# rachtibat/LRP-eXplains-Transformers

Hardware: AMD Instinct MI355X
Metric: explanations/sec (full AttnLRP backward) Llama-3-8B seq=2048 (higher is better)
Workload: dtype bf16

## Files before the change

### include/lrp_hip.h

```cpp
#ifndef LRP_HIP_H
#define LRP_HIP_H
#include <stdint.h>

#ifdef __cplusplus
extern "C" {
#endif

#define LRP_F32 0
#define LRP_BF16 1

#define LRP_OK 0
#define LRP_EINVAL -1
#define LRP_EALIGN -2
#define LRP_ESHAPE -3
#define LRP_ELAUNCH -4

#define LRP_ACT_SILU 0
#define LRP_ACT_GELU_TANH 1
#define LRP_ACT_GELU 2
#define LRP_ACT_TANH 3

int lrp_version(void);
const char* lrp_build_arch(void);
int lrp_last_hip_error(void);
// ... 56 lines not shown
                         float* rel_out, int M, int H, float w_offset, float eps_add,
                         float eps_lin, int dtype, void* stream);

int lrp_sandwich_norm_ok(int H, int dtype);
int lrp_sandwich_norm_fwd(const void* x, const void* res, const void* w_post, const void* w_pre, void* hsum_out, void* y,
                          float* rstd_post, float* rstd_pre, int M, int H, float eps, float w_offset, int dtype, void* stream);
int lrp_sandwich_norm_bwd(const void* Gres, const void* Gx, const void* w_pre, const float* rstd_pre, const void* w_post,
                          const float* rstd_post, void* Gs_out, void* Ga_out, int M, int H, float w_offset, int dtype, void* stream);
int lrp_qk_norm_rope_fwd(const void* qkv, const void* wq, const void* wk, void* qr, void* kr, float* rstd_q, float* rstd_k,
                         const float* cos_t, const float* sin_t, int64_t rows, int seq, int nq, int nk, int d, int64_t ldqkv,
                         int64_t ldq, int64_t ldk, float eps, float w_offset, int dtype, void* stream);
int lrp_qkv_bwd_pack(const void* dq, const void* dk_h, const void* dv_h, const void* wq, const void* wk, const float* rstd_q,
                     const float* rstd_k, const float* cos_t, const float* sin_t, void* A, int64_t rows, int seq, int nq, int nk, int d,
                     int64_t lddq, int64_t lddk, int64_t lddv, int64_t lda, float w_offset, int dtype, void* stream);

int lrp_layernorm_fwd(const void* x, const void* w, const void* b, void* y, float* mean,
                      float* rstd, int M, int H, float eps, int dtype, void* stream);
int lrp_layernorm_bwd(const void* Gy, const void* y, const void* w, const float* rstd,
                      void* Gx, int M, int H, float eps_y, int dtype, void* stream);
int lrp_layernorm_bwd_plain(const void* Gy, const void* x, const void* w, const float* mean, const float* rstd, void* Gx,
                            int M, int H, int dtype, void* stream);


int lrp_gated_act_fwd(const void* g, const void* u, void* m, int M, int I, int64_t ldg,
                      int64_t ldu, int64_t ldm, int act, int dtype, void* stream);
int lrp_gated_act_bwd(const void* Gm, const void* g, const void* u, void* Ag, void* Au,
                      int M, int I, int64_t ldgm, int64_t ldg, int64_t ldu, int64_t ldag,
                      int64_t ldau, float eps_g, float eps_lin, int act, int dtype, void* stream);
#define LRP_GATED_IL 32
int lrp_gated_act_fwd_il(const void* gu, void* m, int M, int I, int64_t ldgu, int64_t ldm, int act, int dtype, void* stream);
int lrp_gated_act_bwd_il(const void* Gm, const void* gu, void* Agu, int M, int I, int64_t ldgm, int64_t ldgu, int64_t ldagu,
                         float eps_g, float eps_lin, int act, int dtype, void* stream);
int lrp_gemm_gated_coef_ok(int M, int I, int H, int64_t ldx, int64_t ldwgu, int64_t lda, int64_t ldwd, int act, int dtype);
int lrp_gemm_gated_fwd_coef(const void* x, const void* Wgu, const float* rs, void* coef, void* m, int M, int I, int K, int64_t ldx, int64_t ldw,
                            int64_t ldcoef, int64_t ldm, float eps_g, float eps_lin, int act, int dtype, void* stream);
int lrp_gemm_gated_bwd_coef(const void* Adn, const void* Wdn, const void* coef, void* Agu, int M, int I, int K, int64_t lda, int64_t ldw,
                            int64_t ldcoef, int64_t ldagu, int dtype, void* stream);

int lrp_gemm_norm_fused_ok(int M, int N, int K, int64_t lda, int64_t ldb, int nn, int dtype);
int lrp_gemm_res_ssq(const void* x, const void* W, const void* res, void* out, float* ssq, int M, int N, int K, int64_t ldx, int64_t ldw,
                     int64_t ldres, int64_t ldout, int64_t ldssq, void* raw, int64_t ldraw, int dtype, void* stream);
int lrp_rms_rstd(const float* ssq, int parts, int64_t ldssq, int M, int H, float eps, float* rstd, void* stream);
int lrp_gemm_nt_rs(const void* x, const void* W, const float* rs, void* out, int M, int N, int K, int64_t ldx, int64_t ldw, int64_t ldout,
                   int dtype, void* stream);
int lrp_gemm_nt_rs_rope_ok(int M, int N, int K, int64_t ldx, int64_t ldw, int64_t ldout, int seq, int rope_cols, int head_dim, int dtype);
int lrp_gemm_nt_rs_rope(const void* x, const void* W, const float* rs, const float* cos, const float* sin, void* out, int M, int N, int K,
                        int64_t ldx, int64_t ldw, int64_t ldout, int seq, int rope_cols, int head_dim, int dtype, void* stream);
int lrp_gemm_nt_rs_bias(const void* x, const void* W, const float* rs, const void* bias, void* out, int M, int N, int K, int64_t ldx, int64_t ldw,
                        int64_t ldout, int dtype, void* stream);
int lrp_gemm_nt_rs_bias_rope_ok(int M, int N, int K, int64_t ldx, int64_t ldw, int64_t ldout, int seq, int rope_cols, int head_dim, int dtype);
int lrp_gemm_nt_rs_bias_rope(const void* x, const void* W, const float* rs, const void* bias, const float* cos, const float* sin, void* out, int M,
                             int N, int K, int64_t ldx, int64_t ldw, int64_t ldout, int seq, int rope_cols, int head_dim, int dtype, void* stream);
int lrp_gemm_nn_rs(const void* s, const void* W, const float* rs, void* out, int M, int N, int K, int64_t lds, int64_t ldw, int64_t ldout,
                   int dtype, void* stream);
int lrp_gemm_nn_rs_res(const void* s, const void* W, const float* rs, const void* res, void* out, int M, int N, int K, int64_t lds, int64_t ldw,
                       int64_t ldres, int64_t ldout, int dtype, void* stream);

int lrp_act_fwd(const void* x, void* y, int64_t n, int act, int dtype, void* stream);
int lrp_act_bwd(const void* Gy, const void* x, void* Gx, int64_t n, float eps_g, int act,
                int dtype, void* stream);
int lrp_act_grad(const void* Gy, const void* x, void* Gx, int64_t n, int act, int dtype, void* stream);

int lrp_add_bcast(const void* x, const void* y, void* out, int M, int H, int period, int dtype, void* stream);

int lrp_rope_fwd(const void* x, void* xr, const float* cos_t, const float* sin_t, int rows,
                 int seq, int n_heads, int d, int64_t ldx, int64_t ldxr, int dtype, void* stream);
int lrp_rope_bwd(const void* Gr, const void* xr, const void* x, void* A, const float* cos_t,
                 const float* sin_t, int rows, int seq, int n_heads, int d, int64_t ldg,
                 int64_t ldxr, int64_t ldx, int64_t lda, float eps_rope, float eps_lin,
                 int dtype, void* stream);

int lrp_transpose_heads(const void* x, void* xt, int B, int S, int H, int d, int64_t ldx,
                        int64_t ldt, int dtype, void* stream);
int lrp_attn_needs_transposed(int dtype, int d);
int lrp_attn_fwd(const void* q, const void* k, const void* v, const void* v_t, void* o, float* lse,
                 int B, int S, int Hq, int Hkv, int d, int64_t ldq, int64_t ldk, int64_t ldv,
                 int64_t ldt, int64_t ldo, float scale, int causal, int window, int q_begin,
                 const int* row_lo, const int* row_hi, int dtype, void* stream);
int lrp_attn_bwd_prep(const void* Go, const void* o, void* Gho, float* D, int B, int S, int Hq,
                      int d, int64_t ldgo, int64_t ldo, int64_t ldgho, float eps_pv,
                      float factor, int dtype, void* stream);
int lrp_attn_bwd_dq(const void* q, const void* k, const void* v, const void* k_t, const void* Gho,
                    const float* lse, const float* D, void* dq, int B, int S, int Hq, int Hkv,
                    int d, int64_t ldq, int64_t ldk, int64_t ldv, int64_t ldt, int64_t ldgho,
                    int64_t lddq, float scale, float eps_mask, float eps_qk, int causal,
                    int window, int q_begin, const int* row_lo, const int* row_hi, int dtype,
                    void* stream);
int lrp_attn_bwd_dq_d_ok(int dtype, int d);
int lrp_attn_bwd_dq_d(const void* q, const void* k, const void* v, const void* Gho, const void* o, const float* lse, float* D, void* dq,
                      int B, int S, int Hq, int Hkv, int d, int64_t ldq, int64_t ldk, int64_t ldv, int64_t ldgho, int64_t ldo, int64_t lddq,
                      float scale, int causal, int window, const int* row_lo, const int* row_hi, const float* cos_t, const float* sin_t,
                      int dtype, void* stream);
int lrp_gqa_reduce_rope(const void* in, void* out, int64_t rows, int seq, int Hkv, int rep, int d, int64_t ld_in, int64_t ld_out,
                        const float* cos_t, const float* sin_t, int dtype, void* stream);
int lrp_attn_bwd_dkv(const void* q, const void* k, const void* v, const void* q_t, const void* Gho,
                     const void* Gho_t, const float* lse, const float* D, void* dk_h, void* dv_h,
                     int B, int S, int Hq, int Hkv, int d, int64_t ldq, int64_t ldk, int64_t ldv,
                     int64_t ldt, int64_t ldgho, int64_t lddk, int64_t lddv, float scale,
                     float eps_mask, float eps_qk, int causal, int window, int q_begin,
                     const int* row_lo, const int* row_hi, int dtype, void* stream);
int lrp_gqa_reduce(const void* in, void* out, int64_t rows, int Hkv, int rep, int d, int64_t ld_in,
                   int64_t ld_out, int dtype, void* stream);

int lrp_softmax_fwd(const void* x, void* p, int64_t rows, int n, float inv_temp, int dtype,
                    void* stream);
int lrp_softmax_rule_bwd(const void* x, const void* p, const void* Rp, void* Rx, int64_t rows,
                         int n, float inv_temp, int dtype, void* stream);
int lrp_add2_rule_bwd(const void* a, const void* b, const void* R, void* Ra, void* Rb,
                      int64_t n, float eps, int dtype, void* stream);

int lrp_readout(const void* emb, const void* G, float* R_tok, int M, int H, int dtype, void* stream);
int64_t lrp_colsum_dot_ws(int B, int S, int N);
int lrp_colsum_dot(const void* x, const void* g, float* out, void* ws, int M, int N, int B, int S, int64_t ldx, int64_t ldg, int dtype,
                   void* stream);
int lrp_head_seed(const void* W_lm, const float* logits, const int* idx, const void* w_norm,
                  const float* rstd_last, void* Gh_last, int B, int V, int H, int64_t ld_logits,
                  float w_offset, float eps_lin, int dtype, void* stream);
int lrp_argmax_rows(const float* logits, int* idx, float* val, int B, int V, int64_t ld, void* stream);
int lrp_transpose(const void* in, void* out, int rows, int cols, int64_t ld_in, int64_t ld_out,
                  int batch, int64_t s_in, int64_t s_out, int dtype, void* stream);
int lrp_cast(const void* in, void* out, int64_t n, int in_dtype, int out_dtype, void* stream);

int64_t lrp_moe_plan_ints(int T, int k, int E);
int lrp_moe_plan(const void* idx, int* plan, int T, int k, int E, void* stream);
int lrp_moe_gate_up_fwd(const void* x, const void* Wgu, const int* plan, void* coef, void* m, int T, int k, int E, int H, int I,
                        int64_t ldx, int64_t ldcoef, int64_t ldm, int act, int dtype, void* stream);
int lrp_moe_down_fwd(const void* m, const void* Wd, const int* plan, void* y, int T, int k, int E, int H, int I, int64_t ldm,
                     int64_t ldy, int dtype, void* stream);
int lrp_moe_combine(const void* rows, const void* w, const int* plan, void* out, int T, int k, int E, int H, int64_t ldr,
                    int64_t ldo, int dtype, void* stream);
int lrp_moe_down_dgrad(const void* G, const void* Wd, const void* coef, const void* m, const void* w, const int* plan, void* Agu,
                       float* gw_part, int T, int k, int E, int H, int I, int64_t ldg, int64_t ldcoef, int64_t ldm,
                       int64_t ldagu, int dtype, void* stream);
int lrp_moe_gw_reduce(const float* gw_part, const int* plan, void* gw, int T, int k, int E, int I, int dtype, void* stream);
int lrp_moe_gate_up_dgrad(const void* Agu, const void* Wgu, const int* plan, void* gx_rows, int T, int k, int E, int H, int I,
                          int64_t ldagu, int64_t ldgx, int dtype, void* stream);

#ifdef __cplusplus
}
#endif
#include "lrp_hip_latent.h"
#include "lrp_hip_moe_router.h"
#include "lrp_hip_mxfp4.h"
#include "lrp_hip_moe_mxfp4.h"
#include "lrp_hip_wgrad.h"
#include "lrp_hip_moe_wgrad.h"
#include "lrp_hip_param_grad.h"
#include "lrp_hip_span.h"
#include "lrp_hip_decode.h"
#include "lrp_hip_decode_site.h"
#include "lrp_hip_mxfp4_stream.h"
#include "lrp_hip_sample.h"
#include "lrp_hip_attn_cp.h"
#endif
```

### lrp-explains-transformers_amd/csrc/attention.hip

```cpp
#include "attention_tiles.hpp"

namespace {

template <typename T, int D, int QSUB>
__global__ __launch_bounds__(ANT, (D >= 256 ? 1 : 2)) void attn_fwd_kernel(
    const T* __restrict__ q, const T* __restrict__ k, const T* __restrict__ vt, T* __restrict__ o, float* __restrict__ lse,
    int S, int Hq, int Hkv, int64_t ldq, int64_t ldk, int64_t ldt, int64_t ldo, float scale, int causal, int window, int q_begin,
    const int* __restrict__ row_lo, const int* __restrict__ row_hi) {
    typedef AT<T> A;
    typedef typename Mma16<T>::frag frag_t;
    constexpr int SZ = A::SZ, CT = A::CT, NC16 = A::NC16, NDC = D * SZ / 64, ND16 = D / 16;
    constexpr int KP = D * SZ;
    constexpr int BQ = 4 * 16 * QSUB;
    extern __shared__ __attribute__((aligned(16))) char smem[];
    char* sK = smem;
    char* sV = smem + CT * KP;

    const int lane = threadIdx.x & 63, wave = threadIdx.x >> 6, g = lane >> 4;
    const int b = blockIdx.z, h = blockIdx.y, hk = h / (Hq / Hkv);
    const int qblk = gridDim.x - 1 - blockIdx.x;
    const int q0 = qblk * BQ, qw = q0 + wave * 16 * QSUB;
    if (q0 + BQ <= q_begin) return;
    const T* qb = q + (int64_t)b * S * ldq + (int64_t)h * D;
    const T* kb = k + (int64_t)b * S * ldk + (int64_t)hk * D;
// ... 872 lines not shown

inline bool al16(const void* p) { return (reinterpret_cast<uintptr_t>(p) & 15) == 0; }

template <auto Kern, typename T, typename... Mid>
void launch_fwd(const AttnCall& c, dim3 grid, int threads, size_t lds, Mid... mid) {
    lrp_launch_lds<Kern>(grid, dim3(threads), lds, lds, c.st, (const T*)c.q, (const T*)c.k, (const T*)c.v_t, (T*)c.o, c.lse_out, c.S, c.Hq, c.Hkv,
                         c.ldq, c.ldk, c.ldt, c.ldo, c.scale, c.causal, c.window, mid..., c.q_begin, c.row_lo, c.row_hi);
}
template <auto Kern, typename T, typename... Mid>
void launch_dq(const AttnCall& c, dim3 grid, int threads, size_t lds, Mid... mid) {
    lrp_launch_lds<Kern>(grid, dim3(threads), lds, lds, c.st, (const T*)c.q, (const T*)c.k, (const T*)c.v, (const T*)c.k_t, (const T*)c.gho, c.lse,
                         c.D, (T*)c.dq, c.S, c.Hq, c.Hkv, c.ldq, c.ldk, c.ldv, c.ldt, c.ldg, c.lddq, c.scale, c.eps_mask, c.eps_qk, c.causal,
                         c.window, mid..., c.q_begin, c.row_lo, c.row_hi);
}
template <auto Kern, typename T, typename... Mid>
void launch_dkv(const AttnCall& c, dim3 grid, int threads, size_t lds, Mid... mid) {
    lrp_launch_lds<Kern>(grid, dim3(threads), lds, lds, c.st, (const T*)c.q, (const T*)c.k, (const T*)c.v, (const T*)c.q_t, (const T*)c.gho,
                         (const T*)c.gho_t, c.lse, c.D, (T*)c.dk, (T*)c.dv, c.S, c.Hq, c.Hkv, c.ldq, c.ldk, c.ldv, c.ldt, c.ldg, c.lddk, c.lddv,
                         c.scale, c.eps_mask, c.eps_qk, c.causal, c.window, mid..., c.q_begin, c.row_lo, c.row_hi);
}

}

static inline bool use_attn32(int dtype, int d) { return dtype == LRP_BF16 && (d == 64 || d == 96 || d == 128 || d == 256); }
extern "C" int lrp_attn_needs_transposed(int dtype, int d) { return use_attn32(dtype, d) ? 0 : 1; }

#define ATT_DISPATCH_D(T, d, ...)                                   \
    if ((size_t)d * sizeof(T) < 64) return LRP_ESHAPE;              \
    if (sizeof(T) == 2 && d != 32) return LRP_ESHAPE;               \
    switch (d) {                                                    \
        case 16: if constexpr (sizeof(T) == 4) { constexpr int DD = 16; __VA_ARGS__ } break;   \
        case 32: { constexpr int DD = 32; __VA_ARGS__ } break;      \
        case 64: if constexpr (sizeof(T) == 4) { constexpr int DD = 64; __VA_ARGS__ } break;   \
        case 128: if constexpr (sizeof(T) == 4) { constexpr int DD = 128; __VA_ARGS__ } break; \
        case 256: if constexpr (sizeof(T) == 4) { constexpr int DD = 256; __VA_ARGS__ } break; \
        default: return LRP_ESHAPE;                                 \
    }

template <typename T> static bool attn_8wave(const AttnCall& c) {
    constexpr int SZ = sizeof(T), CT = 128 / SZ;
    return (c.ldt % CT) == 0 && ((size_t)c.d * SZ >= 64) && c.d <= 128;
}

template <typename T>
static int attn_fwd_t(const AttnCall& c) {
    constexpr int SZ = sizeof(T), CT = 128 / SZ;
    if (attn_8wave<T>(c)) {
        ATT_DISPATCH_D(T, c.d, {
            if constexpr (DD <= 128) {
                const size_t lds = 2 * (2 * (size_t)128 * DD);
                const int rep = c.Hq / c.Hkv;
                if ((int64_t)c.B * c.Hq * ((c.S + 255) / 256) >= 512)
                    launch_fwd<attn_fwd_v2_kernel<T, DD, 2>, T>(c, dim3(xcd_group_grid(c.B * c.Hkv, rep * ((c.S + 255) / 256))), 512, lds, c.B);
                else
                    launch_fwd<attn_fwd_v2_kernel<T, DD, 1>, T>(c, dim3(xcd_group_grid(c.B * c.Hkv, rep * ((c.S + 127) / 128))), 512, lds, c.B);
            }
        })
        return lrp_check_launch();
    }
    ATT_DISPATCH_D(T, c.d, {
        constexpr int QSUB = (DD >= 256) ? 1 : 2;
        constexpr int BQ = 64 * QSUB;
        launch_fwd<attn_fwd_kernel<T, DD, QSUB>, T>(c, dim3((c.S + BQ - 1) / BQ, c.Hq, c.B), ANT, (size_t)CT * DD * SZ + (size_t)DD * 128);
    })
    return lrp_check_launch();
}

static int attn_common_check(int B, int S, int Hq, int Hkv, int d, int dtype, float scale = 1.f) {
    if (!(scale > 0.f)) return LRP_EINVAL;
    if (B < 0 || S < 0 || Hq < 1 || Hkv < 1 || (Hq % Hkv) || d < 16) return LRP_EINVAL;
    if (dtype != LRP_F32 && dtype != LRP_BF16) return LRP_EINVAL;
    if (B > 65535 || Hq > 65535) return LRP_ESHAPE;
    return LRP_OK;
}

extern "C" int lrp_attn_fwd(const void* q, const void* k, const void* v, const void* v_t, void* o, float* lse, int B, int S,
                            int Hq, int Hkv, int d, int64_t ldq, int64_t ldk, int64_t ldv, int64_t ldt, int64_t ldo, float scale,
                            int causal, int window, int q_begin, const int* row_lo, const int* row_hi, int dtype, void* stream) {
    if ((row_lo == nullptr) != (row_hi == nullptr)) return LRP_EINVAL;
    if (!q || !k || !o || !lse) return LRP_EINVAL;
    int rc = attn_common_check(B, S, Hq, Hkv, d, dtype, scale);
    if (rc) return rc;
    if (B == 0 || S == 0) return LRP_OK;
    const int epc = dtype == LRP_F32 ? 4 : 8;
    const bool a32 = use_attn32(dtype, d);
    if (a32) {
        if (!v) return LRP_EINVAL;
        if (!al16(q) || !al16(k) || !al16(v) || !al16(o) || (ldq % epc) || (ldk % epc) || (ldv % epc) || (ldo % 4)) return LRP_EALIGN;
    } else {
        if (!v_t) return LRP_EINVAL;
        if (!al16(q) || !al16(k) || !al16(v_t) || !al16(o) || (ldq % epc) || (ldk % epc) || (ldt % epc) || (ldo % 4) || ldt < S) return LRP_EALIGN;
    }
    AttnCall c = {};
    c.q = q; c.k = k; c.v = v; c.v_t = v_t; c.o = o; c.lse_out = lse;
    c.B = B; c.S = S; c.Hq = Hq; c.Hkv = Hkv; c.d = d;
    c.ldq = ldq; c.ldk = ldk; c.ldv = ldv; c.ldt = ldt; c.ldo = ldo;
    c.scale = scale; c.causal = causal; c.window = window; c.q_begin = q_begin;
    c.row_lo = row_lo; c.row_hi = row_hi; c.st = (hipStream_t)stream;
    if (a32) return lrp_attn32_fwd(c);
    return dtype == LRP_F32 ? attn_fwd_t<float>(c) : attn_fwd_t<bf16_t>(c);
}

template <typename T>
static int attn_dq_t(const AttnCall& c) {
    constexpr int SZ = sizeof(T), CT = 128 / SZ;
    if (attn_8wave<T>(c)) {
        ATT_DISPATCH_D(T, c.d, {
            if constexpr (DD <= 128) {
                const size_t lds = 2 * (3 * (size_t)128 * DD);
                dim3 grid(xcd_group_grid(c.B * c.Hkv, (c.Hq / c.Hkv) * ((c.S + 127) / 128)));
                lrp_with_bool(c.eps_mask != 0.f || c.eps_qk != 0.f, [&](auto ex) {
                    launch_dq<attn_bwd_dq_v2_kernel<T, DD, decltype(ex)::value>, T>(c, grid, 512, lds, c.B);
                });
            }
        })
        return lrp_check_launch();
    }
    ATT_DISPATCH_D(T, c.d, {
        launch_dq<attn_bwd_dq_kernel<T, DD>, T>(c, dim3((c.S + 63) / 64, c.Hq, c.B), ANT, 2 * (size_t)CT * DD * SZ + (size_t)DD * 128);
    })
    return lrp_check_launch();
}

extern "C" int lrp_attn_bwd_dq(const void* q, const void* k, const void* v, const void* k_t, const void* Gho,
                               const float* lse, const float* D, void* dq, int B, int S, int Hq, int Hkv, int d,
                               int64_t ldq, int64_t ldk, int64_t ldv, int64_t ldt, int64_t ldgho, int64_t lddq, float scale,
                               float eps_mask, float eps_qk, int causal, int window, int q_begin, const int* row_lo, const int* row_hi, int dtype, void* stream) {
    if ((row_lo == nullptr) != (row_hi == nullptr)) return LRP_EINVAL;
    if (!q || !k || !v || !Gho || !lse || !D || !dq) return LRP_EINVAL;
    int rc = attn_common_check(B, S, Hq, Hkv, d, dtype, scale);
    if (rc) return rc;
    if (B == 0 || S == 0) return LRP_OK;
    const int epc = dtype == LRP_F32 ? 4 : 8;
    if (!al16(q) || !al16(k) || !al16(v) || !al16(Gho) || !al16(dq) || (ldq % epc) || (ldk % epc) ||
        (ldv % epc) || (ldgho % epc) || (lddq % 4)) return LRP_EALIGN;
    const bool a32 = use_attn32(dtype, d);
    if (!a32) {
        if (!k_t) return LRP_EINVAL;
        if (!al16(k_t) || (ldt % epc) || ldt < S) return LRP_EALIGN;
    }
    AttnCall c = {};
    c.q = q; c.k = k; c.v = v; c.gho = Gho; c.lse = lse; c.D = D;
    c.B = B; c.S = S; c.Hq = Hq; c.Hkv = Hkv; c.d = d;
    c.ldq = ldq; c.ldk = ldk; c.ldv = ldv; c.ldg = ldgho; c.ldt = ldt;
    c.scale = scale; c.eps_mask = eps_mask; c.eps_qk = eps_qk; c.causal = causal; c.window = window; c.q_begin = q_begin;
    c.row_lo = row_lo; c.row_hi = row_hi; c.st = (hipStream_t)stream;
    c.dq = dq; c.lddq = lddq; c.k_t = k_t;
    if (a32) return lrp_attn32_dq(c);
    return dtype == LRP_F32 ? attn_dq_t<float>(c) : attn_dq_t<bf16_t>(c);
}

extern "C" int lrp_attn_bwd_dq_d_ok(int dtype, int d) { return (use_attn32(dtype, d) && d != 256) ? 1 : 0; }

extern "C" int lrp_attn_bwd_dq_d(const void* q, const void* k, const void* v, const void* Gho, const void* o, const float* lse, float* D,
                                 void* dq, int B, int S, int Hq, int Hkv, int d, int64_t ldq, int64_t ldk, int64_t ldv, int64_t ldgho,
                                 int64_t ldo, int64_t lddq, float scale, int causal, int window, const int* row_lo, const int* row_hi,
                                 const float* cos_t, const float* sin_t, int dtype, void* stream) {
    if ((cos_t == nullptr) != (sin_t == nullptr)) return LRP_EINVAL;
    if (cos_t && d != 64 && d != 128) return LRP_ESHAPE;
    if ((row_lo == nullptr) != (row_hi == nullptr)) return LRP_EINVAL;
    if (!q || !k || !v || !Gho || !o || !lse || !D || !dq) return LRP_EINVAL;
    int rc = attn_common_check(B, S, Hq, Hkv, d, dtype, scale);
    if (rc) return rc;
    if (!lrp_attn_bwd_dq_d_ok(dtype, d)) return LRP_ESHAPE;
    if (B == 0 || S == 0) return LRP_OK;
    if (!al16(q) || !al16(k) || !al16(v) || !al16(Gho) || !al16(o) || !al16(dq) || (ldq % 8) || (ldk % 8) || (ldv % 8) || (ldgho % 8) ||
        (ldo % 8) || (lddq % 4)) return LRP_EALIGN;
    AttnCall c = {};
    c.q = q; c.k = k; c.v = v; c.gho = Gho; c.lse = lse; c.D = nullptr;
    c.B = B; c.S = S; c.Hq = Hq; c.Hkv = Hkv; c.d = d;
    c.ldq = ldq; c.ldk = ldk; c.ldv = ldv; c.ldg = ldgho;
    c.scale = scale; c.causal = causal; c.window = window;
    c.row_lo = row_lo; c.row_hi = row_hi; c.st = (hipStream_t)stream;
    c.dq = dq; c.lddq = lddq; c.ofw = o; c.ldo = ldo; c.Dout = D; c.cos_t = cos_t; c.sin_t = sin_t;
    return lrp_attn32_dq(c);
}

template <typename T>
static int attn_dkv_t(const AttnCall& c) {
    constexpr int SZ = sizeof(T), CT = 128 / SZ;
    if (attn_8wave<T>(c) && c.S >= 1) {
        ATT_DISPATCH_D(T, c.d, {
            if constexpr (DD <= 128) {
                const size_t lds = 2 * (4 * (size_t)128 * DD + 512);
                dim3 grid(xcd_group_grid(c.B * c.Hq, (c.S + 127) / 128));
                lrp_with_bool(c.eps_mask != 0.f || c.eps_qk != 0.f, [&](auto ex) {
                    launch_dkv<attn_bwd_dkv_v2_kernel<T, DD, decltype(ex)::value>, T>(c, grid, 512, lds, c.B);
                });
            }
        })
        return lrp_check_launch();
    }
    ATT_DISPATCH_D(T, c.d, {
        launch_dkv<attn_bwd_dkv_kernel<T, DD>, T>(c, dim3((c.S + 63) / 64, c.Hq, c.B), ANT, 2 * (size_t)CT * DD * SZ + 2 * (size_t)DD * 128);
    })
    return lrp_check_launch();
}

extern "C" int lrp_attn_bwd_dkv(const void* q, const void* k, const void* v, const void* q_t, const void* Gho,
                                const void* Gho_t, const float* lse, const float* D, void* dk_h, void* dv_h, int B, int S,
                                int Hq, int Hkv, int d, int64_t ldq, int64_t ldk, int64_t ldv, int64_t ldt, int64_t ldgho,
                                int64_t lddk, int64_t lddv, float scale, float eps_mask, float eps_qk, int causal, int window,
                                int q_begin, const int* row_lo, const int* row_hi, int dtype, void* stream) {
    if ((row_lo == nullptr) != (row_hi == nullptr)) return LRP_EINVAL;
    if (!q || !k || !v || !Gho || !lse || !D || !dk_h || !dv_h) return LRP_EINVAL;
    int rc = attn_common_check(B, S, Hq, Hkv, d, dtype, scale);
    if (rc) return rc;
    if (B == 0 || S == 0) return LRP_OK;
    const int epc = dtype == LRP_F32 ? 4 : 8;
    if (!al16(q) || !al16(k) || !al16(v) || !al16(Gho) || !al16(dk_h) || !al16(dv_h) ||
        (ldq % epc) || (ldk % epc) || (ldv % epc) || (ldgho % epc) || (lddk % 4) || (lddv % 4)) return LRP_EALIGN;
    const bool a32 = use_attn32(dtype, d);
    if (!a32) {
        if (!q_t || !Gho_t) return LRP_EINVAL;
        if (!al16(q_t) || !al16(Gho_t) || (ldt % epc) || ldt < S) return LRP_EALIGN;
    }
    AttnCall c = {};
    c.q = q; c.k = k; c.v = v; c.gho = Gho; c.lse = lse; c.D = D;
    c.B = B; c.S = S; c.Hq = Hq; c.Hkv = Hkv; c.d = d;
    c.ldq = ldq; c.ldk = ldk; c.ldv = ldv; c.ldg = ldgho; c.ldt = ldt;
    c.scale = scale; c.eps_mask = eps_mask; c.eps_qk = eps_qk; c.causal = causal; c.window = window; c.q_begin = q_begin;
    c.row_lo = row_lo; c.row_hi = row_hi; c.st = (hipStream_t)stream;
    c.dk = dk_h; c.dv = dv_h; c.lddk = lddk; c.lddv = lddv; c.q_t = q_t; c.gho_t = Gho_t;
    if (a32) return lrp_attn32_dkv(c);
    return dtype == LRP_F32 ? attn_dkv_t<float>(c) : attn_dkv_t<bf16_t>(c);
}

extern "C" int lrp_transpose_heads(const void* x, void* xt, int B, int S, int H, int d, int64_t ldx, int64_t ldt,
                                   int dtype, void* stream) {
    if (!x || !xt || B < 0 || S < 0 || H < 1 || d < 1 || ldt < S) return LRP_EINVAL;
    if (B == 0 || S == 0) return LRP_OK;
    if ((int64_t)B * H > 65535 || (S + 63) / 64 > 65535) return LRP_ESHAPE;
    hipStream_t st = (hipStream_t)stream;
    dim3 grid((d + 63) / 64, (S + 63) / 64, B * H), block(256);
    const bool vec = dtype == LRP_BF16 && (d % 8) == 0 && (S % 8) == 0 && (ldx % 8) == 0 && (ldt % 8) == 0 && al16(x) && al16(xt);
    if (vec) hipLaunchKernelGGL(transpose_heads_vec_kernel, grid, block, 0, st, (const bf16_t*)x, (bf16_t*)xt, S, H, d, ldx, ldt);
    else if (dtype == LRP_F32) hipLaunchKernelGGL((transpose_heads_kernel<float>), grid, block, 0, st, (const float*)x, (float*)xt, S, H, d, ldx, ldt);
    else if (dtype == LRP_BF16) hipLaunchKernelGGL((transpose_heads_kernel<bf16_t>), grid, block, 0, st, (const bf16_t*)x, (bf16_t*)xt, S, H, d, ldx, ldt);
    else return LRP_EINVAL;
    return lrp_check_launch();
}

extern "C" int lrp_gqa_reduce(const void* in, void* out, int64_t rows, int Hkv, int rep, int d, int64_t ld_in,
                              int64_t ld_out, int dtype, void* stream) {
    if (!in || !out || rows < 0 || Hkv < 1 || rep < 1 || d < 1) return LRP_EINVAL;
    if (rows == 0) return LRP_OK;
    const int epc = dtype == LRP_F32 ? 4 : 8;
    if (dtype != LRP_F32 && dtype != LRP_BF16) return LRP_EINVAL;
    if (!al16(in) || !al16(out) || (d % epc) || (ld_in % epc) || (ld_out % epc)) return LRP_EALIGN;
    hipStream_t st = (hipStream_t)stream;
    const int64_t work = rows * Hkv * (d / epc);
    int64_t nb = (work + 255) / 256;
    if (nb > 2048) nb = 2048;
    if (dtype == LRP_F32) hipLaunchKernelGGL((gqa_reduce_kernel<float>), dim3((unsigned)nb), dim3(256), 0, st, (const float*)in, (float*)out, rows, Hkv, rep, d, ld_in, ld_out);
    else hipLaunchKernelGGL((gqa_reduce_kernel<bf16_t>), dim3((unsigned)nb), dim3(256), 0, st, (const bf16_t*)in, (bf16_t*)out, rows, Hkv, rep, d, ld_in, ld_out);
    return lrp_check_launch();
}

extern "C" int lrp_gqa_reduce_rope(const void* in, void* out, int64_t rows, int seq, int Hkv, int rep, int d, int64_t ld_in, int64_t ld_out,
                                   const float* cos_t, const float* sin_t, int dtype, void* stream) {
    if (!in || !out || !cos_t || !sin_t || rows < 0 || seq < 1 || Hkv < 1 || rep < 1 || d < 2 || (d & 1)) return LRP_EINVAL;
    if (rows == 0) return LRP_OK;
    if (dtype != LRP_F32 && dtype != LRP_BF16) return LRP_EINVAL;
    const int epc = dtype == LRP_F32 ? 4 : 8;
    if (!al16(in) || !al16(out) || ((d / 2) % epc) || (ld_in % epc) || (ld_out % epc)) return LRP_EALIGN;
    hipStream_t st = (hipStream_t)stream;
    const int64_t work = rows * Hkv * (d / 2 / epc);
    int64_t nb = (work + 255) / 256;
    if (nb > 2048) nb = 2048;
    if (dtype == LRP_F32) hipLaunchKernelGGL((gqa_reduce_rope_kernel<float>), dim3((unsigned)nb), dim3(256), 0, st, (const float*)in, (float*)out, rows, seq, Hkv, rep, d, ld_in, ld_out, cos_t, sin_t);
    else hipLaunchKernelGGL((gqa_reduce_rope_kernel<bf16_t>), dim3((unsigned)nb), dim3(256), 0, st, (const bf16_t*)in, (bf16_t*)out, rows, seq, Hkv, rep, d, ld_in, ld_out, cos_t, sin_t);
    return lrp_check_launch();
}
```

### lrp-explains-transformers_amd/csrc/attention32.hip

```cpp
#include "attention32_tiles.hpp"

namespace attn32 {

template <int DH>
__global__ __launch_bounds__(NWQ * 64, 2) void fwd_kernel(
    const bf16_t* __restrict__ q, const bf16_t* __restrict__ k, const bf16_t* __restrict__ v, bf16_t* __restrict__ o,
    float* __restrict__ lse, int S, int Hq, int Hkv, int64_t ldq, int64_t ldk, int64_t ldv, int64_t ldo, float scale,
    int causal, int window, int B, int q_begin, const int* __restrict__ row_lo, const int* __restrict__ row_hi) {
    constexpr int BQ = NWQ * 32, STAGE = 2 * TILE, NK = DH / 16, ND32 = DH / 32;
    extern __shared__ __attribute__((aligned(16))) char smem[];
    const int lane = threadIdx.x & 63, l31 = lane & 31, hi = lane >> 5;
    const int wave = __builtin_amdgcn_readfirstlane(threadIdx.x >> 6);
    const int rep = Hq / Hkv, nqb = (S + BQ - 1) / BQ;
    int bhk, item;
    if (!xcd_group_decode(blockIdx.x, B * Hkv, rep * nqb, bhk, item)) return;
    const int b = bhk / Hkv, hk = bhk % Hkv, h = hk * rep + item % rep;
    const int qblk = nqb - 1 - item / rep;
    const int q0 = qblk * BQ, qw = q0 + wave * 32, qi = qw + l31;
    if (q0 + BQ <= q_begin) return;
    const bf16_t* kb_ = k + (int64_t)b * S * ldk + (int64_t)hk * DH;
    const bf16_t* vb_ = v + (int64_t)b * S * ldv + (int64_t)hk * DH;

    bf16x8 qf[NK];
    load_row_frags<DH>(qf, q + (int64_t)b * S * ldq + (int64_t)h * DH, ldq, qi, S, hi);
    int ivlo = 0, ivhi = S;
    if (row_lo != nullptr && qi < S) { ivlo = row_lo[(int64_t)b * S + qi]; ivhi = row_hi[(int64_t)b * S + qi]; }
    f32x16 oacc[ND32];
#pragma unroll
    for (int db = 0; db < ND32; ++db) oacc[db] = zero16();
    float m_run = -INFINITY, l_run = 0.f;
    const float c1 = scale * LRP_LOG2E;
    int kend = S;
    if (causal) kend = min(S, q0 + BQ);
    int kbeg = 0;
    if (window > 0) { kbeg = q0 - window + 1; kbeg = kbeg < 0 ? 0 : (kbeg / CT) * CT; }
    IvWave ivw = {0, S, 0, S};
    if (row_lo != nullptr) {
        int* ivsh = reinterpret_cast<int*>(smem);
        ivw = iv_wave(ivlo, ivhi, qi < S, wave, ivsh);
        __syncthreads();
        int glo, ghi;
        iv_fold<NWQ>(ivsh, glo, ghi);
        __syncthreads();
        kbeg = max(kbeg, (min(glo, S) / CT) * CT);
        kend = min(kend, ghi);
    }

    auto stage = [&](int kt0, int buf) {
        char* sb = smem + buf * STAGE;
        stage_tile<NWQ, DH>(kb_, ldk, kt0, S, sb, wave, lane);
        stage_tile<NWQ, DH>(vb_, ldv, kt0, S, sb + TILE, wave, lane);
    };
    if (kbeg < kend) stage(kbeg, 0);
    __syncthreads();
    uint32_t arm[NK], atr[NDX][2];
    {
        const uint32_t sbase = lds_addr(smem);
        LaneAddr la;
        la.init(lane);
#pragma unroll
        for (int ks = 0; ks < NK; ++ks) arm[ks] = sbase + la.rm[ks];
#pragma unroll
        for (int db = 0; db < ND32; ++db) { atr[db][0] = sbase + la.tr[db][0]; atr[db][1] = sbase + la.tr[db][1]; }
    }
    int cur = 0;
    for (int kt0 = kbeg; kt0 < kend; kt0 += CT) {
        if (kt0 + CT < kend) stage(kt0 + CT, cur ^ 1);
        const bool dead = (causal && kt0 > qw + 31) || kt0 >= ivw.hi_max || kt0 + CT <= ivw.lo_min;
        if (!dead) {
            f32x16 st[2] = {zero16(), zero16()};
            bf16x8 f0[3], f1[3];
            A32_RD128(f0[0], arm[0], 0); A32_RD128(f1[0], arm[0], 32 * KP);
            A32_RD128(f0[1], arm[1], 0); A32_RD128(f1[1], arm[1], 32 * KP);
            sfor<0, NK>([&](auto ksc) {
                constexpr int ks = decltype(ksc)::value, cu = ks % 3, nx = (ks + 2) % 3;
                if constexpr (ks + 2 < NK) {
                    A32_RD128(f0[nx], arm[ks + 2], 0); A32_RD128(f1[nx], arm[ks + 2], 32 * KP);
                    A32_WAIT(4, "+v"(f0[cu]), "+v"(f1[cu]));
                } else if constexpr (ks + 1 < NK) {
                    A32_WAIT(2, "+v"(f0[cu]), "+v"(f1[cu]));
                } else {
                    A32_WAIT(0, "+v"(f0[cu]), "+v"(f1[cu]));
                }
                st[0] = mfma32(f0[cu], qf[ks], st[0]);
                st[1] = mfma32(f1[cu], qf[ks], st[1]);
                A32_FENCE();
            });
            u32x2 tv0[2][NDX][2], tv1[2][NDX][2];
            tr_group<ND32, TILE>(tv0[0], atr);
            tr_group<ND32, TILE + 16 * KP>(tv0[1], atr);
            A32_FENCE();
            const bool need_mask = (kt0 + CT > S) || (causal && kt0 + CT - 1 > qw) || (window > 0) ||
                                   (row_lo != nullptr && !(kt0 >= ivw.lo_max && kt0 + CT <= ivw.hi_min));
            if (need_mask) {
#pragma unroll
                for (int kb = 0; kb < 2; ++kb)
#pragma unroll
                    for (int r = 0; r < 16; ++r)
                        st[kb][r] = visible(qi, kt0 + kb * 32 + crow(r, hi), S, causal, window, ivlo, ivhi) ? st[kb][r] : -INFINITY;
            }
            float mx = -INFINITY;
#pragma unroll
            for (int kb = 0; kb < 2; ++kb)
#pragma unroll
                for (int r = 0; r < 16; ++r) mx = fmaxf(mx, st[kb][r]);
            mx = half_max(mx);
            float m_new = m_run;
            if (__any((mx - m_run) * c1 > 8.f || (m_run == -INFINITY && mx != -INFINITY))) m_new = fmaxf(m_run, mx);
            const float m_use = (m_new == -INFINITY) ? 0.f : m_new;
            const float nm2 = -m_use * c1;
            float rs = 0.f;
#pragma unroll
            for (int kb = 0; kb < 2; ++kb)
#pragma unroll
                for (int r = 0; r < 16; ++r) {
                    const float p = fast_exp2(__builtin_fmaf(st[kb][r], c1, nm2));
                    st[kb][r] = p;
                    rs += p;
                }
            rs = half_sum(rs);
            if (__any(m_new != m_run)) {
                const float alpha = fast_exp2((m_run - m_use) * c1);
                l_run = l_run * alpha + rs;
#pragma unroll
                for (int db = 0; db < ND32; ++db) oacc[db] *= alpha;
            } else l_run += rs;
            m_run = m_new;
            const bf16x8 p00 = pack8(st[0], 0), p01 = pack8(st[0], 1), p10 = pack8(st[1], 0), p11 = pack8(st[1], 1);
            A32_FENCE();
            tr_group<ND32, TILE + 32 * KP>(tv1[0], atr);
            wait_tr2<ND32, 2 * ND32>(tv0[0], tv0[1]);
#pragma unroll
            for (int db = 0; db < ND32; ++db) oacc[db] = mfma32(join_tr(tv0[0][db][0], tv0[0][db][1]), p00, oacc[db]);
            A32_FENCE();
            tr_group<ND32, TILE + 48 * KP>(tv1[1], atr);
#pragma unroll
            for (int db = 0; db < ND32; ++db) oacc[db] = mfma32(join_tr(tv0[1][db][0], tv0[1][db][1]), p01, oacc[db]);
            A32_FENCE();
            wait_tr<ND32, 2 * ND32>(tv1[0]);
#pragma unroll
            for (int db = 0; db < ND32; ++db) oacc[db] = mfma32(join_tr(tv1[0][db][0], tv1[0][db][1]), p10, oacc[db]);
            A32_FENCE();
            wait_tr<ND32, 0>(tv1[1]);
#pragma unroll
            for (int db = 0; db < ND32; ++db) oacc[db] = mfma32(join_tr(tv1[1][db][0], tv1[1][db][1]), p11, oacc[db]);
            A32_FENCE();
        }
        asm volatile("s_waitcnt vmcnt(0)" ::: "memory");
        __syncthreads();
        {
            const uint32_t delta = cur ? (uint32_t)-STAGE : (uint32_t)STAGE;
#pragma unroll
            for (int ks = 0; ks < NK; ++ks) arm[ks] += delta;
#pragma unroll
            for (int db = 0; db < ND32; ++db) { atr[db][0] += delta; atr[db][1] += delta; }
        }
        cur ^= 1;
    }
    const float inv = (l_run > 0.f) ? 1.f / l_run : 0.f;
    store_rows<DH>(o + (int64_t)b * S * ldo + (int64_t)h * DH, ldo, qi, S, oacc, inv, hi);
    if (hi == 0 && qi < S) lse[((int64_t)b * Hq + h) * S + qi] = m_run * scale + __logf(l_run);
}

template <bool EXPL, int DH>
__global__ __launch_bounds__(NWQ * 64, 2) void dq_kernel(
    const bf16_t* __restrict__ q, const bf16_t* __restrict__ k, const bf16_t* __restrict__ v, const bf16_t* __restrict__ gho,
    const float* __restrict__ lse, const float* __restrict__ Dd, bf16_t* __restrict__ dq, int S, int Hq, int Hkv, int64_t ldq,
    int64_t ldk, int64_t ldv, int64_t ldg, int64_t lddq, float scale, float eps_mask, float eps_qk, int causal, int window,
    int B, int q_begin, const int* __restrict__ row_lo, const int* __restrict__ row_hi, const bf16_t* __restrict__ ofw, int64_t ldo,
    float* __restrict__ Dout, const float* __restrict__ rope_cos, const float* __restrict__ rope_sin) {
    constexpr int BQ = NWQ * 32, STAGE = 2 * TILE, NK = DH / 16, ND32 = DH / 32;
    extern __shared__ __attribute__((aligned(16))) char smem[];
    const int lane = threadIdx.x & 63, l31 = lane & 31, hi = lane >> 5;
    const int wave = __builtin_amdgcn_readfirstlane(threadIdx.x >> 6);
    const int rep = Hq / Hkv, nqb = (S + BQ - 1) / BQ;
    int bhk, item;
    if (!xcd_group_decode(blockIdx.x, B * Hkv, rep * nqb, bhk, item)) return;
    const int b = bhk / Hkv, hk = bhk % Hkv, h = hk * rep + item % rep;
    const int qblk = nqb - 1 - item / rep;
    const int q0 = qblk * BQ, qw = q0 + wave * 32, qi = qw + l31;
    if (q0 + BQ <= q_begin) return;
    const bf16_t* kb_ = k + (int64_t)b * S * ldk + (int64_t)hk * DH;
    const bf16_t* vb_ = v + (int64_t)b * S * ldv + (int64_t)hk * DH;

    bf16x8 qf[NK], gf[NK];
    load_row_frags<DH>(qf, q + (int64_t)b * S * ldq + (int64_t)h * DH, ldq, qi, S, hi);
    load_row_frags<DH>(gf, gho + (int64_t)b * S * ldg + (int64_t)h * DH, ldg, qi, S, hi);
    const float lse2 = ((qi < S) ? lse[((int64_t)b * Hq + h) * S + qi] : 0.f) * LRP_LOG2E;
    float Dq;
    if (ofw != nullptr) {
        bf16x8 of[NK];
        load_row_frags<DH>(of, ofw + (int64_t)b * S * ldo + (int64_t)h * DH, ldo, qi, S, hi);
        float sd = 0.f;
#pragma unroll
        for (int ks = 0; ks < NK; ++ks)
#pragma unroll
            for (int e = 0; e < 8; ++e) sd += (float)gf[ks][e] * (float)of[ks][e];
        sd += __shfl_xor(sd, 32);
        Dq = sd;
        if (hi == 0 && qi < S) Dout[((int64_t)b * Hq + h) * S + qi] = sd;
    } else Dq = (qi < S) ? Dd[((int64_t)b * Hq + h) * S + qi] : 0.f;
    int ivlo = 0, ivhi = S;
    if (row_lo != nullptr && qi < S) { ivlo = row_lo[(int64_t)b * S + qi]; ivhi = row_hi[(int64_t)b * S + qi]; }
    f32x16 acc[ND32];
#pragma unroll
    for (int db = 0; db < ND32; ++db) acc[db] = zero16();
    const float c1 = scale * LRP_LOG2E;
    int kend = S;
    if (causal) kend = min(S, q0 + BQ);
    int kbeg = 0;
    if (window > 0) { kbeg = q0 - window + 1; kbeg = kbeg < 0 ? 0 : (kbeg / CT) * CT; }
    IvWave ivw = {0, S, 0, S};
    if (row_lo != nullptr) {
        int* ivsh = reinterpret_cast<int*>(smem);
        ivw = iv_wave(ivlo, ivhi, qi < S, wave, ivsh);
        __syncthreads();
        int glo, ghi;
        iv_fold<NWQ>(ivsh, glo, ghi);
        __syncthreads();
        kbeg = max(kbeg, (min(glo, S) / CT) * CT);
        kend = min(kend, ghi);
    }

    auto stage = [&](int kt0, int buf) {
        char* sb = smem + buf * STAGE;
        stage_tile<NWQ, DH>(kb_, ldk, kt0, S, sb, wave, lane);
        stage_tile<NWQ, DH>(vb_, ldv, kt0, S, sb + TILE, wave, lane);
    };
    if (kbeg < kend) stage(kbeg, 0);
    __syncthreads();
    uint32_t arm[NK], atr[NDX][2];
    {
        const uint32_t sbase = lds_addr(smem);
        LaneAddr la;
        la.init(lane);
#pragma unroll
        for (int ks = 0; ks < NK; ++ks) arm[ks] = sbase + la.rm[ks];
#pragma unroll
        for (int db = 0; db < ND32; ++db) { atr[db][0] = sbase + la.tr[db][0]; atr[db][1] = sbase + la.tr[db][1]; }
    }
#ifdef A32_TIMELINE
    uint32_t tl_acc[8] = {0, 0, 0, 0, 0, 0, 0, 0}, tl_prev = (uint32_t)__builtin_readcyclecounter();
    const uint32_t tl_start = tl_prev;
#endif
    int cur = 0;
    for (int kt0 = kbeg; kt0 < kend; kt0 += CT) {
        if (kt0 + CT < kend) stage(kt0 + CT, cur ^ 1);
        A32_TS(0);
        sfor<0, 2>([&](auto kbc) {
            constexpr int kb = decltype(kbc)::value, KO = kb * 32 * KP;
            const int kk0 = kt0 + kb * 32;
            if ((causal && kk0 > qw + 31) || kk0 >= S || kk0 >= ivw.hi_max || kk0 + 32 <= ivw.lo_min) return;
            f32x16 st = zero16(), dp = zero16();
            bf16x8 fk[3], fv[3];
            A32_RD128(fk[0], arm[0], KO); A32_RD128(fv[0], arm[0], KO + TILE);
            A32_RD128(fk[1], arm[1], KO); A32_RD128(fv[1], arm[1], KO + TILE);
            sfor<0, NK>([&](auto ksc) {
                constexpr int ks = decltype(ksc)::value, cu = ks % 3, nx = (ks + 2) % 3;
                if constexpr (ks + 2 < NK) {
                    A32_RD128(fk[nx], arm[ks + 2], KO); A32_RD128(fv[nx], arm[ks + 2], KO + TILE);
                    A32_WAIT(4, "+v"(fk[cu]), "+v"(fv[cu]));
                } else if constexpr (ks + 1 < NK) {
                    A32_WAIT(2, "+v"(fk[cu]), "+v"(fv[cu]));
                } else {
                    A32_WAIT(0, "+v"(fk[cu]), "+v"(fv[cu]));
                }
                st = mfma32(fk[cu], qf[ks], st);
                dp = mfma32(fv[cu], gf[ks], dp);
                A32_FENCE();
            });
            A32_TS(1);
            u32x2 tk[2][NDX][2];
            tr_group<ND32, KO>(tk[0], atr);
            tr_group<ND32, KO + 16 * KP>(tk[1], atr);
            A32_FENCE();
            const bool masked = (kk0 + 32 > S) || (causal && kk0 + 31 > qw) || (window > 0) ||
                                (row_lo != nullptr && !(kk0 >= ivw.lo_max && kk0 + 32 <= ivw.hi_min));
            if (masked) {
#pragma unroll
                for (int r = 0; r < 16; ++r) {
                    const float s_raw = st[r];
                    float p = fast_exp2(__builtin_fmaf(s_raw, c1, -lse2));
                    if (!visible(qi, kk0 + crow(r, hi), S, causal, window, ivlo, ivhi)) p = 0.f;
                    st[r] = lrp_ds<EXPL>(s_raw, p, dp[r], Dq, scale, eps_mask, eps_qk);
                }
            } else {
#pragma unroll
                for (int r = 0; r < 16; ++r) {
                    const float s_raw = st[r];
                    const float p = fast_exp2(__builtin_fmaf(s_raw, c1, -lse2));
                    st[r] = lrp_ds<EXPL>(s_raw, p, dp[r], Dq, scale, eps_mask, eps_qk);
                }
            }
            const bf16x8 df0 = pack8(st, 0), df1 = pack8(st, 1);
            A32_FENCE();
            A32_TS(2);
            wait_tr<ND32, 2 * ND32>(tk[0]);
#pragma unroll
            for (int db = 0; db < ND32; ++db) acc[db] = mfma32(join_tr(tk[0][db][0], tk[0][db][1]), df0, acc[db]);
            A32_FENCE();
            wait_tr<ND32, 0>(tk[1]);
#pragma unroll
            for (int db = 0; db < ND32; ++db) acc[db] = mfma32(join_tr(tk[1][db][0], tk[1][db][1]), df1, acc[db]);
            A32_FENCE();
            A32_TS(3);
        });
        asm volatile("s_waitcnt vmcnt(0)" ::: "memory");
        A32_TS(4);
        __syncthreads();
        A32_TS(5);
        {
            const uint32_t delta = cur ? (uint32_t)-STAGE : (uint32_t)STAGE;
#pragma unroll
            for (int ks = 0; ks < NK; ++ks) arm[ks] += delta;
#pragma unroll
            for (int db = 0; db < ND32; ++db) { atr[db][0] += delta; atr[db][1] += delta; }
        }
        cur ^= 1;
    }
    const float omul = EXPL ? 1.f : 0.5f * scale;
    if constexpr (!EXPL && (DH == 64 || DH == 128)) {
        if (rope_cos != nullptr) {
            const int pos = qi < S ? qi : 0;
            const float* pc = rope_cos + (int64_t)pos * DH;
            const float* ps = rope_sin + (int64_t)pos * DH;
#pragma unroll
            for (int db = 0; db < ND32 / 2; ++db)
#pragma unroll
                for (int i = 0; i < 4; ++i) {
                    const int c = db * 32 + 8 * i + 4 * hi;
                    const f32x4 c1 = *reinterpret_cast<const f32x4*>(pc + c), s1 = *reinterpret_cast<const f32x4*>(ps + c);
#pragma unroll
                    for (int e = 0; e < 4; ++e) {
                        const float g1 = acc[db][4 * i + e], g2 = acc[db + ND32 / 2][4 * i + e];
                        acc[db][4 * i + e] = g1 * c1[e] + g2 * s1[e];
                        acc[db + ND32 / 2][4 * i + e] = g2 * c1[e] - g1 * s1[e];
                    }
                }
        }
    }
    store_rows<DH>(dq + (int64_t)b * S * lddq + (int64_t)h * DH, lddq, qi, S, acc, omul, hi);
#ifdef A32_TIMELINE
    if (lane == 0 && qw < S) {
        uint32_t* w = reinterpret_cast<uint32_t*>(dq + ((int64_t)b * S + qw) * lddq + (int64_t)h * DH);
#pragma unroll
        for (int i = 0; i < 6; ++i) w[i] = tl_acc[i];
        w[6] = (uint32_t)__builtin_readcyclecounter() - tl_start;
        w[7] = (uint32_t)((kend - kbeg + CT - 1) / CT);
    }
#endif
}

template <bool EXPL, int DH, bool IV>
__global__ __launch_bounds__(512, 2) void dkv_kernel(
    const bf16_t* __restrict__ q, const bf16_t* __restrict__ k, const bf16_t* __restrict__ v, const bf16_t* __restrict__ gho,
    const float* __restrict__ lse, const float* __restrict__ Dd, bf16_t* __restrict__ dk, bf16_t* __restrict__ dv, int S, int Hq,
    int Hkv, int64_t ldq, int64_t ldk, int64_t ldv, int64_t ldg, int64_t lddk, int64_t lddv, float scale, float eps_mask,
    float eps_qk, int causal, int window, int B, int q_begin, const int* __restrict__ row_lo, const int* __restrict__ row_hi) {
    constexpr int BK = NW * 32, STAGE = 2 * TILE + 512, VROWS = 32 * KP, NK = DH / 16, ND32 = DH / 32;
    extern __shared__ __attribute__((aligned(16))) char smem[];
    const int lane = threadIdx.x & 63, l31 = lane & 31, hi = lane >> 5;
    const int wave = __builtin_amdgcn_readfirstlane(threadIdx.x >> 6);
    int bh, kblk;
    if (!xcd_item_major_decode(blockIdx.x, B * Hq, (S + BK - 1) / BK, bh, kblk)) return;
    const int b = bh / Hq, h = bh % Hq, hk = h / (Hq / Hkv);
    const int k0 = kblk * BK, kw = k0 + wave * 32, ki = kw + l31;
    const bf16_t* qb_ = q + (int64_t)b * S * ldq + (int64_t)h * DH;
    const bf16_t* gb_ = gho + (int64_t)b * S * ldg + (int64_t)h * DH;
    const float* lse_b = lse + ((int64_t)b * Hq + h) * S;
    const float* D_b = Dd + ((int64_t)b * Hq + h) * S;
    const int* rlo_b = (IV && row_lo) ? row_lo + (int64_t)b * S : nullptr;
    const int* rhi_b = (IV && row_lo) ? row_hi + (int64_t)b * S : nullptr;
    int* const ivtab = reinterpret_cast<int*>(smem + 2 * STAGE + NW * VROWS);

    bf16x8 kf[NK];
    load_row_frags<DH>(kf, k + (int64_t)b * S * ldk + (int64_t)hk * DH, ldk, ki, S, hi);
    char* sVw = smem + 2 * STAGE + wave * VROWS;
    {
        const bf16_t* vbase = v + (int64_t)b * S * ldv + (int64_t)hk * DH;
        const __amdgpu_buffer_rsrc_t rs = __builtin_amdgcn_make_buffer_rsrc((void*)vbase, 0, (int)(((int64_t)(S - 1) * ldv + DH) * 2), 0x00020000);
        const int rl = lane >> 4, slot = lane & 15;
#pragma unroll
        for (int g = 0; g < 8; ++g) {
            const int chunk_ = slot ^ ((rl << 2) | (g & 3));
            const int voff = (DH == 128 || chunk_ < DH / 8) ? (int)(rl * ldv * 2) + (chunk_ << 4) : A32_OOB;
            __builtin_amdgcn_raw_ptr_buffer_load_lds(rs, (lds_ptr_t)(sVw + g * 1024), 16, voff, (int)((int64_t)(kw + g * 4) * ldv * 2), 0, 0);
        }
    }
    f32x16 dkacc[ND32], dvacc[ND32];
#pragma unroll
    for (int db = 0; db < ND32; ++db) { dkacc[db] = zero16(); dvacc[db] = zero16(); }
    const float c1 = scale * LRP_LOG2E;
    int qbeg = 0, qend = S;
    if (causal) qbeg = (k0 / CT) * CT;
    if (window > 0) qend = min(S, k0 + BK - 1 + window);
    if (q_begin > qbeg) qbeg = (q_begin / CT) * CT;
    if (rlo_b != nullptr) {
        int qlo, qhi;
        iv_block_table<NW>(rlo_b, rhi_b, S, k0, BK, wave, lane, ivtab, reinterpret_cast<int*>(smem), qlo, qhi);
        qbeg = max(qbeg, (min(qlo, S) / CT) * CT);
        qend = min(qend, qhi);
    }

    auto stage = [&](int qt0, int buf) {
        char* sb = smem + buf * STAGE;
        stage_tile<NW, DH>(qb_, ldq, qt0, S, sb, wave, lane);
        stage_tile<NW, DH>(gb_, ldg, qt0, S, sb + TILE, wave, lane);
        if (wave == 0) stage_stats(lse_b, qt0, S, sb + 2 * TILE, lane);
        if (wave == 1) stage_stats(D_b, qt0, S, sb + 2 * TILE + 256, lane);
    };
    if (qbeg < qend) stage(qbeg, 0);
    __syncthreads();
    uint32_t arm0, avw0, atr[ND32][2], ast;
    {
        const uint32_t sbase = lds_addr(smem);
        LaneAddr la;
        la.init(lane);
        arm0 = sbase + la.rm[0];
        avw0 = arm0 + 2 * STAGE + wave * VROWS;
#pragma unroll
        for (int db = 0; db < ND32; ++db) { atr[db][0] = sbase + la.tr[db][0]; atr[db][1] = sbase + la.tr[db][1]; }
        ast = sbase + 2 * TILE + hi * 16;
    }
#ifdef A32_TIMELINE
    uint32_t tl_acc[8] = {0, 0, 0, 0, 0, 0, 0, 0}, tl_prev = (uint32_t)__builtin_readcyclecounter();
    const uint32_t tl_start = tl_prev;
#endif
    int cur = 0;
    for (int qt0 = qbeg; qt0 < qend; qt0 += CT) {
        if (qt0 + CT < qend) stage(qt0 + CT, cur ^ 1);
        A32_TS(0);
        sfor<0, 2>([&](auto qbc) {
            constexpr int qb = decltype(qbc)::value, QO = qb * 32 * KP, SO = qb * 128;
            const int qq0 = qt0 + qb * 32;
            bool live = !((causal && qq0 + 31 < kw) || qq0 >= S);
            bool iv_mask = false;
            if (live && rlo_b != nullptr) {
                int t0_, t1_, t2_, t3_;
                iv_row(ivtab, qq0 >> 5, t0_, t1_, t2_, t3_);
                if (t1_ <= kw || t0_ >= kw + 32) live = false;
                iv_mask = !(t2_ <= kw && t3_ >= kw + 32);
            }
            if (!live) return;
            f32x16 st = zero16(), dp = zero16();
            f32x4 sl[2], sd[2];
            constexpr int PD = 2, RS = PD + 1;
            bf16x8 fq[RS], fg[RS], fv[RS];
            static_assert(PD < NK, "read-ahead deeper than the contraction");
            static_assert(PD == 2, "the prologue below issues the reads of steps 0 .. PD - 1");
#define A32_P1_PRO(pk)                                                                                          \
    {                                                                                                           \
        const uint32_t aq = frag_addr<(pk)>(arm0), av = frag_addr<(pk)>(avw0);                                  \
        A32_RD128(fq[pk], aq, QO); A32_RD128(fg[pk], aq, QO + TILE); A32_RD128(fv[pk], av, 0);                  \
    }
            A32_P1_PRO(0) A32_P1_PRO(1)
#undef A32_P1_PRO
            sfor<0, NK>([&](auto ksc) {
                constexpr int ks = decltype(ksc)::value, cu = ks % RS, nx = (ks + PD) % RS;
                constexpr int ahead = (ks + PD < NK ? PD : NK - 1 - ks);
                if constexpr (ks + PD < NK) {
                    const uint32_t aq = frag_addr<ks + PD>(arm0), av = frag_addr<ks + PD>(avw0);
                    A32_RD128(fq[nx], aq, QO); A32_RD128(fg[nx], aq, QO + TILE); A32_RD128(fv[nx], av, 0);
                }
                if constexpr (ks == NK - 2) { A32_RD128(sl[0], ast, SO); A32_RD128(sd[0], ast, SO + 256); }
                constexpr int nw = 3 * ahead + (ks >= NK - 2 ? 2 : 0);
                static_assert(nw <= 14, "lgkmcnt is a 4-bit counter");
                asm volatile("s_waitcnt lgkmcnt(%[n])" : "+v"(fq[cu]), "+v"(fg[cu]), "+v"(fv[cu]) : [n] "n"(nw));
                st = mfma32(fq[cu], kf[ks], st);
                dp = mfma32(fg[cu], fv[cu], dp);
                A32_FENCE();
            });
            A32_TS(1);
            u32x2 tg[2][2], tq[2][2];
#define A32_TRG(slot, jj, dbb)                                                                                        \
    A32_RDTR(tg[slot][0], atr[dbb][0], QO + TILE + (jj) * 16 * KP); A32_RDTR(tg[slot][1], atr[dbb][1], QO + TILE + (jj) * 16 * KP); \
    A32_RDTR(tq[slot][0], atr[dbb][0], QO + (jj) * 16 * KP); A32_RDTR(tq[slot][1], atr[dbb][1], QO + (jj) * 16 * KP)
#define A32_TIE(sl_) "+v"(tg[sl_][0]), "+v"(tg[sl_][1]), "+v"(tq[sl_][0]), "+v"(tq[sl_][1])
#define A32_DKV_STEP(g, wait_stmt)                                                                     \
    {                                                                                                  \
        constexpr int j_ = (g) / ND32, db_ = (g) % ND32, sl_ = (g)&1;                                  \
        wait_stmt;                                                                                     \
        dvacc[db_] = mfma32(join_tr(tg[sl_][0], tg[sl_][1]), pf[j_], dvacc[db_]);                      \
        dkacc[db_] = mfma32(join_tr(tq[sl_][0], tq[sl_][1]), df[j_], dkacc[db_]);                      \
        A32_FENCE();                                                                                   \
    }
            const bool masked = (qq0 + 32 > S) || (causal && qq0 < kw + 31) || (window > 0) || iv_mask;
            bf16x8 pf[2], df[2];
            auto elementwise = [&](auto ic) {
                constexpr int i = decltype(ic)::value, cu = i & 1, nx = cu ^ 1;
                if constexpr (i == 0) {
                    A32_RD128(sl[nx], ast, SO + 32); A32_RD128(sd[nx], ast, SO + 32 + 256);
                    A32_WAIT(6, "+v"(sl[cu]), "+v"(sd[cu]));
                } else if constexpr (i == 1) {
                    A32_RD128(sl[nx], ast, SO + 64); A32_RD128(sd[nx], ast, SO + 64 + 256);
                    A32_WAIT(2, "+v"(sl[cu]), "+v"(sd[cu]), A32_TIE(0));
                } else if constexpr (i == 2) {
                    A32_RD128(sl[nx], ast, SO + 96); A32_RD128(sd[nx], ast, SO + 96 + 256);
                    A32_WAIT(6, "+v"(sl[cu]), "+v"(sd[cu]));
                } else if constexpr (ND32 == 3) {
                    A32_WAIT(0, "+v"(sl[cu]), "+v"(sd[cu]), A32_TIE(1));
                } else {
                    A32_WAIT(0, "+v"(sl[cu]), "+v"(sd[cu]), A32_TIE(0));
                }
                float pe[4];
#pragma unroll
                for (int e = 0; e < 4; ++e) pe[e] = fast_exp2(__builtin_fmaf(st[4 * i + e], c1, -(sl[cu][e] * LRP_LOG2E)));
                if (masked) {
#pragma unroll
                    for (int e = 0; e < 4; ++e) {
                        const int qi = qq0 + 8 * i + 4 * hi + e;
                        int ivlo = 0, ivhi = S;
                        if constexpr (IV) { if (rlo_b != nullptr && qi < S) { ivlo = rlo_b[qi]; ivhi = rhi_b[qi]; } }
                        pe[e] = ((qi < S) & visible(qi, ki, S, causal, window, ivlo, ivhi)) ? pe[e] : 0.f;
                    }
                }
#pragma unroll
                for (int e = 0; e < 4; ++e) {
                    const int r = 4 * i + e;
                    pf[i >> 1][4 * (i & 1) + e] = (bf16_t)pe[e];
                    df[i >> 1][4 * (i & 1) + e] = (bf16_t)lrp_ds<EXPL>(st[r], pe[e], dp[r], sd[cu][e], scale, eps_mask, eps_qk);
                }
                A32_FENCE();
            };
            A32_TRG(0, 0, 0);
            A32_FENCE();
            elementwise(IC<0>{});
            elementwise(IC<1>{});
            if constexpr (ND32 == 4) {
                A32_TS(2);
                A32_TRG(1, 0, 1);
                A32_DKV_STEP(0, (void)0);
                A32_TRG(0, 0, 2);
                A32_DKV_STEP(1, A32_WAIT(4, A32_TIE(1)));
                A32_TRG(1, 0, 3);
                A32_DKV_STEP(2, A32_WAIT(4, A32_TIE(0)));
                A32_TRG(0, 1, 0);
                A32_DKV_STEP(3, A32_WAIT(4, A32_TIE(1)));
                A32_TS(3);
                elementwise(IC<2>{});
                elementwise(IC<3>{});
                A32_TS(2);
                A32_TRG(1, 1, 1);
                A32_DKV_STEP(4, (void)0);
                A32_TRG(0, 1, 2);
                A32_DKV_STEP(5, A32_WAIT(4, A32_TIE(1)));
                A32_TRG(1, 1, 3);
                A32_DKV_STEP(6, A32_WAIT(4, A32_TIE(0)));
                A32_DKV_STEP(7, A32_WAIT(0, A32_TIE(1)));
                A32_TS(3);
            } else if constexpr (ND32 == 3) {
                A32_TRG(1, 0, 1);
                A32_DKV_STEP(0, (void)0);
                A32_TRG(0, 0, 2);
                A32_DKV_STEP(1, A32_WAIT(4, A32_TIE(1)));
                A32_TRG(1, 1, 0);
                A32_DKV_STEP(2, A32_WAIT(4, A32_TIE(0)));
                elementwise(IC<2>{});
                elementwise(IC<3>{});
                A32_TRG(0, 1, 1);
                A32_DKV_STEP(3, (void)0);
                A32_TRG(1, 1, 2);
                A32_DKV_STEP(4, A32_WAIT(4, A32_TIE(0)));
                A32_DKV_STEP(5, A32_WAIT(0, A32_TIE(1)));
            } else {
                A32_TRG(1, 0, 1);
                A32_DKV_STEP(0, (void)0);
                A32_TRG(0, 1, 0);
                A32_DKV_STEP(1, A32_WAIT(4, A32_TIE(1)));
                elementwise(IC<2>{});
                elementwise(IC<3>{});
                A32_TRG(1, 1, 1);
                A32_DKV_STEP(2, (void)0);
                A32_DKV_STEP(3, A32_WAIT(0, A32_TIE(1)));
            }
#undef A32_DKV_STEP
#undef A32_TIE
#undef A32_TRG
        });
        asm volatile("s_waitcnt vmcnt(0)" ::: "memory");
        A32_TS(4);
        __syncthreads();
        A32_TS(5);
        {
            const uint32_t delta = cur ? (uint32_t)-STAGE : (uint32_t)STAGE;
            arm0 += delta;
#pragma unroll
            for (int db = 0; db < ND32; ++db) { atr[db][0] += delta; atr[db][1] += delta; }
            ast += delta;
        }
        cur ^= 1;
    }
    store_rows<DH>(dk + (int64_t)b * S * lddk + (int64_t)h * DH, lddk, ki, S, dkacc, EXPL ? 1.f : 0.5f * scale, hi);
    store_rows<DH>(dv + (int64_t)b * S * lddv + (int64_t)h * DH, lddv, ki, S, dvacc, 1.f, hi);
#ifdef A32_TIMELINE
    asm volatile("s_waitcnt vmcnt(0)" ::: "memory");
    if (lane == 0 && kw < S) {
        uint32_t* w = reinterpret_cast<uint32_t*>(dk + ((int64_t)b * S + kw) * lddk + (int64_t)h * DH);
#pragma unroll
        for (int i = 0; i < 6; ++i) w[i] = tl_acc[i];
        w[6] = (uint32_t)__builtin_readcyclecounter() - tl_start;
        w[7] = (uint32_t)((qend - qbeg + CT - 1) / CT);
    }
#endif
}


namespace d256 {

constexpr int D2 = 256, KP2 = 512, CT2 = 32, TILE2 = CT2 * KP2, NK2 = 16, ND2 = 8, NW2 = 4;

LRP_DEVICE void stage_tile2(const bf16_t* base, int64_t ld, int row0, int S, char* lds, int wave, int lane) {
    const __amdgpu_buffer_rsrc_t rs = __builtin_amdgcn_make_buffer_rsrc((void*)base, 0, (int)(((int64_t)(S - 1) * ld + D2) * 2), 0x00020000);
    const int rl = lane >> 5, slot = lane & 31;
#pragma unroll
    for (int g = 0; g < 4; ++g) {
        const int grp = g * NW2 + wave;
        const int rot = ((2 * (wave & 1) + rl) << 2) | ((2 * g + (wave >> 1)) & 3);
        const int voff = (int)(rl * ld * 2) + ((slot ^ rot) << 4);
        __builtin_amdgcn_raw_ptr_buffer_load_lds(rs, (lds_ptr_t)(lds + grp * 1024), 16, voff, (int)((int64_t)(row0 + 2 * grp) * ld * 2), 0, 0);
    }
}
LRP_DEVICE void stage_block2(const bf16_t* base, int64_t ld, int row0, int S, char* lds, int lane) {
    const __amdgpu_buffer_rsrc_t rs = __builtin_amdgcn_make_buffer_rsrc((void*)base, 0, (int)(((int64_t)(S - 1) * ld + D2) * 2), 0x00020000);
    const int rl = lane >> 5, slot = lane & 31;
#pragma unroll
    for (int g = 0; g < 16; ++g) {
        const int rot = ((2 * (g & 1) + rl) << 2) | ((g >> 1) & 3);
        const int voff = (int)(rl * ld * 2) + ((slot ^ rot) << 4);
        __builtin_amdgcn_raw_ptr_buffer_load_lds(rs, (lds_ptr_t)(lds + g * 1024), 16, voff, (int)((int64_t)(row0 + 2 * g) * ld * 2), 0, 0);
    }
}
LRP_DEVICE uint32_t rm_base(int lane) {
    const int l31 = lane & 31, hi = lane >> 5;
    return (uint32_t)(l31 * KP2 + ((hi ^ rot4(l31)) << 4));
}
LRP_DEVICE uint32_t tr_base(int lane, int half) {
    const int l31 = lane & 31, hi = lane >> 5, i16 = lane & 15;
    const int r = half * 8 + 4 * hi + (i16 >> 2);
    const int chunk = ((l31 >> 4) << 1) + ((i16 & 3) >> 1);
    return (uint32_t)(r * KP2 + ((chunk ^ rot4(r)) << 4) + 8 * (i16 & 1));
}
template <int X> LRP_DEVICE uint32_t xor_addr(uint32_t a0) {
    if constexpr (X == 0) return a0;
    else {
        uint32_t r;
        asm volatile("v_xor_b32 %0, %1, %2" : "=v"(r) : "n"(X), "v"(a0));
        return r;
    }
}
LRP_DEVICE void load_row_frags2(bf16x8* f, const bf16_t* base, int64_t ld, int row, int S, int hi) {
    const bool ok = row < S;
#pragma unroll
    for (int ks = 0; ks < NK2; ++ks) {
        if (ok) f[ks] = *reinterpret_cast<const bf16x8*>(base + (int64_t)row * ld + ks * 16 + hi * 8);
        else {
            u32x4 z = {0, 0, 0, 0};
            f[ks] = __builtin_bit_cast(bf16x8, z);
        }
    }
}
LRP_DEVICE void store_rows2(bf16_t* base, int64_t ld, int row, int S, const f32x16* acc, float mul, int hi) {
    attn32::store_rows<D2>(base, ld, row, S, acc, mul, hi);
}
#define A2_UNIT(dst, a0, a1, J, DBH, OFF)                                                                            \
    {                                                                                                                \
        const uint32_t b0_ = xor_addr<((DBH) * 4 + 0) << 6>(a0), c0_ = xor_addr<((DBH) * 4 + 0) << 6>(a1);           \
        const uint32_t b1_ = xor_addr<((DBH) * 4 + 1) << 6>(a0), c1_ = xor_addr<((DBH) * 4 + 1) << 6>(a1);           \
        const uint32_t b2_ = xor_addr<((DBH) * 4 + 2) << 6>(a0), c2_ = xor_addr<((DBH) * 4 + 2) << 6>(a1);           \
        const uint32_t b3_ = xor_addr<((DBH) * 4 + 3) << 6>(a0), c3_ = xor_addr<((DBH) * 4 + 3) << 6>(a1);           \
        A32_RDTR(dst[0][0], b0_, (OFF) + (J) * 16 * KP2); A32_RDTR(dst[0][1], c0_, (OFF) + (J) * 16 * KP2);          \
        A32_RDTR(dst[1][0], b1_, (OFF) + (J) * 16 * KP2); A32_RDTR(dst[1][1], c1_, (OFF) + (J) * 16 * KP2);          \
        A32_RDTR(dst[2][0], b2_, (OFF) + (J) * 16 * KP2); A32_RDTR(dst[2][1], c2_, (OFF) + (J) * 16 * KP2);          \
        A32_RDTR(dst[3][0], b3_, (OFF) + (J) * 16 * KP2); A32_RDTR(dst[3][1], c3_, (OFF) + (J) * 16 * KP2);          \
    }
#define A2_UNITV(t) "+v"(t[0][0]), "+v"(t[0][1]), "+v"(t[1][0]), "+v"(t[1][1]), "+v"(t[2][0]), "+v"(t[2][1]), "+v"(t[3][0]), "+v"(t[3][1])

__global__ __launch_bounds__(NW2 * 64, 1) void fwd256_kernel(
    const bf16_t* __restrict__ q, const bf16_t* __restrict__ k, const bf16_t* __restrict__ v, bf16_t* __restrict__ o,
    float* __restrict__ lse, int S, int Hq, int Hkv, int64_t ldq, int64_t ldk, int64_t ldv, int64_t ldo, float scale,
    int causal, int window, int B, int q_begin, const int* __restrict__ row_lo, const int* __restrict__ row_hi) {
    constexpr int BQ = NW2 * 32, STAGE = 2 * TILE2;
    extern __shared__ __attribute__((aligned(16))) char smem[];
    const int lane = threadIdx.x & 63, l31 = lane & 31, hi = lane >> 5;
    const int wave = __builtin_amdgcn_readfirstlane(threadIdx.x >> 6);
    const int rep = Hq / Hkv, nqb = (S + BQ - 1) / BQ;
    int bhk, item;
    if (!xcd_group_decode(blockIdx.x, B * Hkv, rep * nqb, bhk, item)) return;
    const int b = bhk / Hkv, hk = bhk % Hkv, h = hk * rep + item % rep;
    const int qblk = nqb - 1 - item / rep;
    const int q0 = qblk * BQ, qw = q0 + wave * 32, qi = qw + l31;
    if (q0 + BQ <= q_begin) return;
    const bf16_t* kb_ = k + (int64_t)b * S * ldk + (int64_t)hk * D2;
    const bf16_t* vb_ = v + (int64_t)b * S * ldv + (int64_t)hk * D2;

    bf16x8 qf[NK2];
    load_row_frags2(qf, q + (int64_t)b * S * ldq + (int64_t)h * D2, ldq, qi, S, hi);
    int ivlo = 0, ivhi = S;
    if (row_lo != nullptr && qi < S) { ivlo = row_lo[(int64_t)b * S + qi]; ivhi = row_hi[(int64_t)b * S + qi]; }
    f32x16 oacc[ND2];
#pragma unroll
    for (int db = 0; db < ND2; ++db) oacc[db] = zero16();
    float m_run = -INFINITY, l_run = 0.f;
    const float c1 = scale * LRP_LOG2E;
    int kend = S;
    if (causal) kend = min(S, q0 + BQ);
    int kbeg = 0;
    if (window > 0) { kbeg = q0 - window + 1; kbeg = kbeg < 0 ? 0 : (kbeg / CT2) * CT2; }
    IvWave ivw = {0, S, 0, S};
    if (row_lo != nullptr) {
        int* ivsh = reinterpret_cast<int*>(smem);
        ivw = iv_wave(ivlo, ivhi, qi < S, wave, ivsh);
        __syncthreads();
        int glo, ghi;
        iv_fold<NW2>(ivsh, glo, ghi);
        __syncthreads();
        kbeg = max(kbeg, (min(glo, S) / CT2) * CT2);
        kend = min(kend, ghi);
    }

    auto stage = [&](int kt0, int buf) {
        char* sb = smem + buf * STAGE;
        stage_tile2(kb_, ldk, kt0, S, sb, wave, lane);
        stage_tile2(vb_, ldv, kt0, S, sb + TILE2, wave, lane);
    };
    if (kbeg < kend) stage(kbeg, 0);
    asm volatile("s_waitcnt vmcnt(0)" ::: "memory");
    __syncthreads();
    uint32_t arm = lds_addr(smem) + rm_base(lane), at0 = lds_addr(smem) + tr_base(lane, 0), at1 = lds_addr(smem) + tr_base(lane, 1);
    int cur = 0;
    for (int kt0 = kbeg; kt0 < kend; kt0 += CT2) {
        if (kt0 + CT2 < kend) stage(kt0 + CT2, cur ^ 1);
        const bool dead = (causal && kt0 > qw + 31) || (window > 0 && kt0 + CT2 - 1 <= qw - window) || kt0 >= ivw.hi_max || kt0 + CT2 <= ivw.lo_min;
        if (!dead) {
            f32x16 st = zero16();
            bf16x8 fk[3];
            A32_RD128(fk[0], arm, 0);
            { const uint32_t a_ = xor_addr<1 << 5>(arm); A32_RD128(fk[1], a_, 0); }
            sfor<0, NK2>([&](auto ksc) {
                constexpr int ks = decltype(ksc)::value, cu = ks % 3, nx = (ks + 2) % 3;
                (void)&fk; (void)&arm;
                if constexpr (ks + 2 < NK2) {
                    { const uint32_t a_ = xor_addr<(ks + 2) << 5>(arm); A32_RD128(fk[nx], a_, 0); }
                    A32_WAIT(2, "+v"(fk[cu]));
                } else if constexpr (ks + 1 < NK2) {
// ... 277 lines not shown
                iv_mask = !(t2_ <= kw && t3_ >= kw + 32);
            }
            if (!dead) {
                f32x16 st = zero16(), dp = zero16();
                bf16x8 fq[3];
                A32_RD128(fq[0], arm, 0);
                { const uint32_t a_ = xor_addr<1 << 5>(arm); A32_RD128(fq[1], a_, 0); }
                sfor<0, NK2>([&](auto ksc) {
                    constexpr int ks = decltype(ksc)::value, cu = ks % 3, nx = (ks + 2) % 3;
                    (void)&fq; (void)&arm;
                    if constexpr (ks + 2 < NK2) {
                        { const uint32_t a_ = xor_addr<(ks + 2) << 5>(arm); A32_RD128(fq[nx], a_, 0); }
                        A32_WAIT(2, "+v"(fq[cu]));
                    } else if constexpr (ks + 1 < NK2) {
                        A32_WAIT(1, "+v"(fq[cu]));
                    } else {
                        A32_WAIT(0, "+v"(fq[cu]));
                    }
                    st = mfma32(fq[cu], kf[ks], st);
                    A32_FENCE();
                });
                if constexpr (PASS == 1) {
                    bf16x8 fg[3], fv[3];
                    A32_RD128(fg[0], arm, TILE2); A32_RD128(fv[0], avw, 0);
                    { const uint32_t a_ = xor_addr<1 << 5>(arm), b_ = xor_addr<1 << 5>(avw); A32_RD128(fg[1], a_, TILE2); A32_RD128(fv[1], b_, 0); }
                    sfor<0, NK2>([&](auto ksc) {
                        constexpr int ks = decltype(ksc)::value, cu = ks % 3, nx = (ks + 2) % 3;
                        (void)&fg; (void)&fv; (void)&arm; (void)&avw;
                        if constexpr (ks + 2 < NK2) {
                            { const uint32_t a_ = xor_addr<(ks + 2) << 5>(arm), b_ = xor_addr<(ks + 2) << 5>(avw); A32_RD128(fg[nx], a_, TILE2); A32_RD128(fv[nx], b_, 0); }
                            A32_WAIT(4, "+v"(fg[cu]), "+v"(fv[cu]));
                        } else if constexpr (ks + 1 < NK2) {
                            A32_WAIT(2, "+v"(fg[cu]), "+v"(fv[cu]));
                        } else {
                            A32_WAIT(0, "+v"(fg[cu]), "+v"(fv[cu]));
                        }
                        dp = mfma32(fg[cu], fv[cu], dp);
                        A32_FENCE();
                    });
                }
                constexpr int TOFF = (PASS == 0) ? TILE2 : 0;
                u32x2 tt[2][4][2];
                A2_UNIT(tt[0], at0, at1, 0, 0, TOFF);
                A32_FENCE();
                const bool masked = (qt0 + 32 > S) || (causal && qt0 < kw + 31) || (window > 0 && qt0 + 31 - window >= kw) || iv_mask;
                bf16x8 xf[2];
                f32x4 sl[2], sd[2];
                sfor<0, 2>([&](auto jc) {
                    constexpr int j = decltype(jc)::value;
                    (void)&sl; (void)&sd; (void)&ast;
                    A32_RD128(sl[0], ast, 64 * j); A32_RD128(sl[1], ast, 64 * j + 32);
                    if constexpr (PASS == 1) {
                        A32_RD128(sd[0], ast, 64 * j + 256); A32_RD128(sd[1], ast, 64 * j + 32 + 256);
                        A32_WAIT(0, "+v"(sl[0]), "+v"(sl[1]), "+v"(sd[0]), "+v"(sd[1]));
                    } else {
                        A32_WAIT(0, "+v"(sl[0]), "+v"(sl[1]));
                    }
#pragma unroll
                    for (int ii = 0; ii < 2; ++ii)
#pragma unroll
                        for (int e = 0; e < 4; ++e) {
                            const int i = 2 * j + ii, r = 4 * i + e;
                            const float s_raw = st[r];
                            float p = fast_exp2(__builtin_fmaf(s_raw, c1, -(sl[ii][e] * LRP_LOG2E)));
                            if (masked) {
                                const int qi = qt0 + 8 * i + 4 * hi + e;
                                int ivlo = 0, ivhi = S;
                                if (rlo_b != nullptr && qi < S) { ivlo = rlo_b[qi]; ivhi = rhi_b[qi]; }
                                p = ((qi < S) & visible(qi, ki, S, causal, window, ivlo, ivhi)) ? p : 0.f;
                            }
                            if constexpr (PASS == 0) xf[j][4 * ii + e] = (bf16_t)p;
                            else xf[j][4 * ii + e] = (bf16_t)lrp_ds<EXPL>(s_raw, p, dp[r], sd[ii][e], scale, eps_mask, eps_qk);
                        }
                    A32_FENCE();
                });
                A2_UNIT(tt[1], at0, at1, 0, 1, TOFF);
                A32_WAIT(8, A2_UNITV(tt[0]));
#pragma unroll
                for (int d4 = 0; d4 < 4; ++d4) acc[d4] = mfma32(join_tr(tt[0][d4][0], tt[0][d4][1]), xf[0], acc[d4]);
                A32_FENCE();
                A2_UNIT(tt[0], at0, at1, 1, 0, TOFF);
                A32_WAIT(8, A2_UNITV(tt[1]));
#pragma unroll
                for (int d4 = 0; d4 < 4; ++d4) acc[4 + d4] = mfma32(join_tr(tt[1][d4][0], tt[1][d4][1]), xf[0], acc[4 + d4]);
                A32_FENCE();
                A2_UNIT(tt[1], at0, at1, 1, 1, TOFF);
                A32_WAIT(8, A2_UNITV(tt[0]));
#pragma unroll
                for (int d4 = 0; d4 < 4; ++d4) acc[d4] = mfma32(join_tr(tt[0][d4][0], tt[0][d4][1]), xf[1], acc[d4]);
                A32_FENCE();
                A32_WAIT(0, A2_UNITV(tt[1]));
#pragma unroll
                for (int d4 = 0; d4 < 4; ++d4) acc[4 + d4] = mfma32(join_tr(tt[1][d4][0], tt[1][d4][1]), xf[1], acc[4 + d4]);
                A32_FENCE();
            }
            asm volatile("s_waitcnt vmcnt(0)" ::: "memory");
            __syncthreads();
            {
                const uint32_t delta = cur ? (uint32_t)-STAGE : (uint32_t)STAGE;
                arm += delta; at0 += delta; at1 += delta; ast += delta;
            }
            cur ^= 1;
        }
        if constexpr (PASS == 0) store_rows2(dv + (int64_t)b * S * lddv + (int64_t)h * D2, lddv, ki, S, acc, 1.f, hi);
        else store_rows2(dk + (int64_t)b * S * lddk + (int64_t)h * D2, lddk, ki, S, acc, EXPL ? 1.f : 0.5f * scale, hi);
    });
}

}

constexpr size_t A32_LDS_MAX = 160 * 1024;

template <auto Kern>
static void launch_fwd(const AttnCall& c, int nw, size_t lds) {
    dim3 grid(xcd_group_grid(c.B * c.Hkv, (c.Hq / c.Hkv) * ((c.S + nw * 32 - 1) / (nw * 32))));
    lrp_launch_lds<Kern>(grid, dim3(nw * 64), lds, lds, c.st, (const bf16_t*)c.q, (const bf16_t*)c.k, (const bf16_t*)c.v, (bf16_t*)c.o, c.lse_out,
                         c.S, c.Hq, c.Hkv, c.ldq, c.ldk, c.ldv, c.ldo, c.scale, c.causal, c.window, c.B, c.q_begin, c.row_lo, c.row_hi);
}
template <auto Kern, typename... Tail>
static void launch_dq(const AttnCall& c, int nw, size_t lds, Tail... tail) {
    dim3 grid(xcd_group_grid(c.B * c.Hkv, (c.Hq / c.Hkv) * ((c.S + nw * 32 - 1) / (nw * 32))));
    lrp_launch_lds<Kern>(grid, dim3(nw * 64), lds, lds, c.st, (const bf16_t*)c.q, (const bf16_t*)c.k, (const bf16_t*)c.v, (const bf16_t*)c.gho,
                         c.lse, c.D, (bf16_t*)c.dq, c.S, c.Hq, c.Hkv, c.ldq, c.ldk, c.ldv, c.ldg, c.lddq, c.scale, c.eps_mask, c.eps_qk,
                         c.causal, c.window, c.B, c.q_begin, c.row_lo, c.row_hi, tail...);
}
template <auto Kern>
static void launch_dkv(const AttnCall& c, int nw, size_t lds) {
    dim3 grid(xcd_group_grid(c.B * c.Hq, (c.S + nw * 32 - 1) / (nw * 32)));
    lrp_launch_lds<Kern>(grid, dim3(nw * 64), lds, A32_LDS_MAX, c.st, (const bf16_t*)c.q, (const bf16_t*)c.k, (const bf16_t*)c.v,
                         (const bf16_t*)c.gho, c.lse, c.D, (bf16_t*)c.dk, (bf16_t*)c.dv, c.S, c.Hq, c.Hkv, c.ldq, c.ldk, c.ldv, c.ldg, c.lddk,
                         c.lddv, c.scale, c.eps_mask, c.eps_qk, c.causal, c.window, c.B, c.q_begin, c.row_lo, c.row_hi);
}

}

#define A32_FOR_DH(d, ...)                                     \
    switch (d) {                                               \
        case 64: { constexpr int DH = 64; __VA_ARGS__ } break; \
        case 96: { constexpr int DH = 96; __VA_ARGS__ } break; \
        case 128: { constexpr int DH = 128; __VA_ARGS__ } break; \
        default: return LRP_ESHAPE;                            \
    }

int lrp_attn32_fwd(const AttnCall& c) {
    using namespace attn32;
    if (c.d == 256) launch_fwd<d256::fwd256_kernel>(c, d256::NW2, 2 * (2 * (size_t)d256::TILE2));
    else A32_FOR_DH(c.d, { launch_fwd<fwd_kernel<DH>>(c, NWQ, 2 * (2 * (size_t)TILE)); })
    return lrp_check_launch();
}

int lrp_attn32_dq(const AttnCall& c) {
    using namespace attn32;
    const bool expl = c.eps_mask != 0.f || c.eps_qk != 0.f;
    if (c.d == 256)
        lrp_with_bool(expl, [&](auto ex) { launch_dq<d256::dq256_kernel<decltype(ex)::value>>(c, d256::NW2, 2 * (2 * (size_t)d256::TILE2)); });
    else A32_FOR_DH(c.d, {
        lrp_with_bool(expl, [&](auto ex) {
            launch_dq<dq_kernel<decltype(ex)::value, DH>>(c, NWQ, 2 * (2 * (size_t)TILE), (const bf16_t*)c.ofw, c.ldo, c.Dout, c.cos_t, c.sin_t);
        });
    })
    return lrp_check_launch();
}

int lrp_attn32_dkv(const AttnCall& c) {
    using namespace attn32;
    const bool wide = c.d == 256, expl = c.eps_mask != 0.f || c.eps_qk != 0.f, iv = c.row_lo != nullptr;
    const size_t lds = (wide ? 2 * (2 * (size_t)d256::TILE2 + 512) + (size_t)d256::NW2 * 32 * d256::KP2 : 2 * (2 * (size_t)TILE + 512) + (size_t)NW * 32 * KP) +
                       (iv ? (size_t)((c.S + 31) / 32) * 16 : 0);
    if (lds > A32_LDS_MAX) return LRP_ESHAPE;
    if (wide) lrp_with_bool(expl, [&](auto ex) { launch_dkv<d256::dkv256_kernel<decltype(ex)::value>>(c, d256::NW2, lds); });
    else A32_FOR_DH(c.d, {
        lrp_with_bool(expl, [&](auto ex) {
            lrp_with_bool(iv, [&](auto ivf) { launch_dkv<dkv_kernel<decltype(ex)::value, DH, decltype(ivf)::value>>(c, NW, lds); });
        });
    })
    return lrp_check_launch();
}
```

### lrp-explains-transformers_amd/csrc/attention32_tiles.hpp

```cpp
#pragma once
#include "common.hpp"

namespace attn32 {

typedef __attribute__((ext_vector_type(4))) short s16x4;
typedef __attribute__((address_space(3))) s16x4* lds_s16x4_t;
typedef __attribute__((address_space(3))) void* lds_ptr_t;
typedef const __attribute__((address_space(1))) void* glb_ptr_t;

constexpr int NW = 8;
constexpr int NWQ = 4;
constexpr int CT = 64;
constexpr int KP = 256;
constexpr int TILE = CT * KP;
constexpr int NKX = 8, NDX = 4;
#define LRP_LOG2E 1.4426950408889634f

LRP_DEVICE int rot4(int r) { return ((r & 3) << 2) | ((r >> 2) & 3); }
LRP_DEVICE float fast_exp2(float x) { return __builtin_amdgcn_exp2f(x); }

LRP_DEVICE bool xcd_group_decode(int L, int ngroups, int per_group, int& group, int& item) {
    const int xcd = L & 7, i = L >> 3;
    item = i % per_group;
    group = xcd + 8 * (i / per_group);
    return group < ngroups;
}
LRP_DEVICE bool xcd_item_major_decode(int L, int ngroups, int per_group, int& group, int& item) {
    const int xcd = L & 7, i = L >> 3, gpx = (ngroups + 7) >> 3;
    item = i / gpx;
    group = xcd + 8 * (i % gpx);
    return group < ngroups;
}

constexpr int A32_OOB = 0x40000000;
template <int NWV = NW, int DH = 128>
LRP_DEVICE void stage_tile(const bf16_t* base, int64_t ld, int row0, int S, char* lds, int wave, int lane) {
    const __amdgpu_buffer_rsrc_t rs = __builtin_amdgcn_make_buffer_rsrc((void*)base, 0, (int)(((int64_t)(S - 1) * ld + DH) * 2), 0x00020000);
    const int rl = lane >> 4, slot = lane & 15;
    const int chunk_ = slot ^ ((rl << 2) | (wave & 3));
    const int voff = (DH == 128 || chunk_ < DH / 8) ? (int)(rl * ld * 2) + (chunk_ << 4) : A32_OOB;
#pragma unroll
    for (int g = 0; g < 16 / NWV; ++g) {
        const int grp = g * NWV + wave;
        __builtin_amdgcn_raw_ptr_buffer_load_lds(rs, (lds_ptr_t)(lds + grp * 1024), 16, voff, (int)((int64_t)(row0 + grp * 4) * ld * 2), 0, 0);
    }
}
LRP_DEVICE void stage_stats(const float* base, int r0, int S, char* lds, int lane) {
    int r = r0 + lane;
    r = r < S ? r : S - 1;
    __builtin_amdgcn_global_load_lds((glb_ptr_t)(base + r), (lds_ptr_t)lds, 4, 0, 0);
}

struct LaneAddr {
    uint32_t rm[NKX];
    uint32_t tr[NDX][2];
    LRP_DEVICE void init(int lane) {
        const int l31 = lane & 31, hi = lane >> 5, i16 = lane & 15;
#pragma unroll
        for (int ks = 0; ks < NKX; ++ks) rm[ks] = l31 * KP + (((ks * 2 + hi) ^ rot4(l31)) << 4);
#pragma unroll
        for (int db = 0; db < NDX; ++db)
#pragma unroll
            for (int half = 0; half < 2; ++half) {
                const int r = half * 8 + 4 * hi + (i16 >> 2);
                const int chunk = db * 4 + ((l31 >> 4) << 1) + ((i16 & 3) >> 1);
                tr[db][half] = r * KP + ((chunk ^ rot4(r)) << 4) + 8 * (i16 & 1);
            }
    }
};

LRP_DEVICE bf16x8 lds_frag(const char* tile, uint32_t off) { return *reinterpret_cast<const bf16x8*>(tile + off); }
LRP_DEVICE bf16x8 lds_frag_tr(const char* tile, uint32_t off0, uint32_t off1) {
    const s16x4 a = __builtin_amdgcn_ds_read_tr16_b64_v4i16((lds_s16x4_t)(tile + off0));
    const s16x4 b = __builtin_amdgcn_ds_read_tr16_b64_v4i16((lds_s16x4_t)(tile + off1));
    typedef __attribute__((ext_vector_type(8))) short s16x8;
    const s16x8 v = {a[0], a[1], a[2], a[3], b[0], b[1], b[2], b[3]};
    return __builtin_bit_cast(bf16x8, v);
}
LRP_DEVICE f32x16 mfma32(bf16x8 a, bf16x8 b, f32x16 c) { return __builtin_amdgcn_mfma_f32_32x32x16_bf16(a, b, c, 0, 0, 0); }
LRP_DEVICE f32x16 zero16() {
    f32x16 z;
#pragma unroll
    for (int i = 0; i < 16; ++i) z[i] = 0.f;
    return z;
}
LRP_DEVICE bf16x8 pack8(const f32x16& x, int j) {
    bf16x8 r;
#pragma unroll
    for (int e = 0; e < 8; ++e) r[e] = (bf16_t)x[8 * j + e];
    return r;
}
LRP_DEVICE int crow(int r, int hi) { return (r & 3) + 8 * (r >> 2) + 4 * hi; }

#define A32_RD128(dst, addr, off) asm volatile("ds_read_b128 %0, %1 offset:%2" : "=&v"(dst) : "v"(addr), "n"(off))
#define A32_RDTR(dst, addr, off) asm volatile("ds_read_b64_tr_b16 %0, %1 offset:%2" : "=&v"(dst) : "v"(addr), "n"(off))
#define A32_WAIT(n, ...) asm volatile("s_waitcnt lgkmcnt(" #n ")" : __VA_ARGS__)
#define A32_FENCE() __builtin_amdgcn_sched_barrier(0)
template <int ND, int OFF> LRP_DEVICE void tr_group(u32x2 (&dst)[NDX][2], const uint32_t (&adr)[NDX][2]) {
    A32_RDTR(dst[0][0], adr[0][0], OFF); A32_RDTR(dst[0][1], adr[0][1], OFF);
    A32_RDTR(dst[1][0], adr[1][0], OFF); A32_RDTR(dst[1][1], adr[1][1], OFF);
    if constexpr (ND > 2) { A32_RDTR(dst[2][0], adr[2][0], OFF); A32_RDTR(dst[2][1], adr[2][1], OFF); }
    if constexpr (ND > 3) { A32_RDTR(dst[3][0], adr[3][0], OFF); A32_RDTR(dst[3][1], adr[3][1], OFF); }
}
#define A32_TRV2(t) "+v"(t[0][0]), "+v"(t[0][1]), "+v"(t[1][0]), "+v"(t[1][1])
#define A32_TRV3(t) A32_TRV2(t), "+v"(t[2][0]), "+v"(t[2][1])
#define A32_TRV4(t) A32_TRV3(t), "+v"(t[3][0]), "+v"(t[3][1])
template <int ND, int N> LRP_DEVICE void wait_tr(u32x2 (&t)[NDX][2]) {
    if constexpr (ND == 4) asm volatile("s_waitcnt lgkmcnt(%[n])" : A32_TRV4(t) : [n] "n"(N));
    else if constexpr (ND == 3) asm volatile("s_waitcnt lgkmcnt(%[n])" : A32_TRV3(t) : [n] "n"(N));
    else asm volatile("s_waitcnt lgkmcnt(%[n])" : A32_TRV2(t) : [n] "n"(N));
}
template <int ND, int N> LRP_DEVICE void wait_tr2(u32x2 (&t)[NDX][2], u32x2 (&u)[NDX][2]) {
    if constexpr (ND == 4) asm volatile("s_waitcnt lgkmcnt(%[n])" : A32_TRV4(t), A32_TRV4(u) : [n] "n"(N));
    else if constexpr (ND == 3) asm volatile("s_waitcnt lgkmcnt(%[n])" : A32_TRV3(t), A32_TRV3(u) : [n] "n"(N));
    else asm volatile("s_waitcnt lgkmcnt(%[n])" : A32_TRV2(t), A32_TRV2(u) : [n] "n"(N));
}
#ifdef A32_TIMELINE
#define A32_TS(slot)                                                          \
    {                                                                         \
        asm volatile("s_waitcnt lgkmcnt(0)" ::: "memory");                    \
        const uint32_t now_ = (uint32_t)__builtin_readcyclecounter();         \
        tl_acc[slot] += now_ - tl_prev;                                       \
        tl_prev = now_;                                                       \
    }
#else
#define A32_TS(slot)
#endif
template <int V> struct IC { static constexpr int value = V; };
template <int I, int N, typename F> LRP_DEVICE void sfor(F&& f) {
    if constexpr (I < N) {
        f(IC<I>{});
        sfor<I + 1, N>(static_cast<F&&>(f));
    }
}
LRP_DEVICE void half_swap(float& a, float& b) { asm volatile("s_nop 1\n\tv_permlane32_swap_b32 %0, %1" : "+v"(a), "+v"(b)); }
LRP_DEVICE float half_max(float x) {
    float a = x, b = x;
    half_swap(a, b);
    return fmaxf(a, b);
}
LRP_DEVICE float half_sum(float x) {
    float a = x, b = x;
    half_swap(a, b);
    return a + b;
}
template <int KS> LRP_DEVICE uint32_t frag_addr(uint32_t a0) {
    if constexpr (KS == 0) return a0;
    else {
        uint32_t r;
        asm volatile("v_xor_b32 %0, %1, %2" : "=v"(r) : "n"(KS << 5), "v"(a0));
        return r;
    }
}
LRP_DEVICE uint32_t lds_addr(const void* p) { return (uint32_t)(uintptr_t)(lds_ptr_t)p; }
LRP_DEVICE bf16x8 join_tr(u32x2 a, u32x2 b) {
    const u32x4 v = {a[0], a[1], b[0], b[1]};
    return __builtin_bit_cast(bf16x8, v);
}

template <int DH>
LRP_DEVICE void load_row_frags(bf16x8* f, const bf16_t* base, int64_t ld, int row, int S, int hi) {
    const bool ok = row < S;
#pragma unroll
    for (int ks = 0; ks < DH / 16; ++ks) {
        if (ok) f[ks] = *reinterpret_cast<const bf16x8*>(base + (int64_t)row * ld + ks * 16 + hi * 8);
        else {
            u32x4 z = {0, 0, 0, 0};
            f[ks] = __builtin_bit_cast(bf16x8, z);
        }
    }
}
template <int DH>
LRP_DEVICE void store_rows(bf16_t* base, int64_t ld, int row, int S, const f32x16* acc, float mul, int hi) {
    const bool wide = (((reinterpret_cast<uintptr_t>(base) | (uintptr_t)(ld * 2)) & 15) == 0);
    if (!wide) {
        if (row >= S) return;
#pragma unroll
        for (int db = 0; db < DH / 32; ++db)
#pragma unroll
            for (int i = 0; i < 4; ++i) {
                bf16x4 v;
#pragma unroll
                for (int e = 0; e < 4; ++e) v[e] = (bf16_t)(acc[db][4 * i + e] * mul);
                *reinterpret_cast<bf16x4*>(base + (int64_t)row * ld + db * 32 + 8 * i + 4 * hi) = v;
            }
        return;
    }
    bf16_t* const rb = base + (int64_t)row * ld + 8 * hi;
#pragma unroll
    for (int db = 0; db < DH / 32; ++db)
#pragma unroll
        for (int i = 0; i < 4; i += 2) {
            bf16x4 va, vb;
#pragma unroll
            for (int e = 0; e < 4; ++e) { va[e] = (bf16_t)(acc[db][4 * i + e] * mul); vb[e] = (bf16_t)(acc[db][4 * (i + 1) + e] * mul); }
            u32x2 a = __builtin_bit_cast(u32x2, va), b = __builtin_bit_cast(u32x2, vb);
            auto r0 = __builtin_amdgcn_permlane32_swap(a[0], b[0], false, false);
            auto r1 = __builtin_amdgcn_permlane32_swap(a[1], b[1], false, false);
            const u32x4 o = {r0[0], r1[0], r0[1], r1[1]};
            if (row < S) *reinterpret_cast<u32x4*>(rb + db * 32 + 8 * i) = o;
        }
}

LRP_DEVICE bool visible(int q, int key, int S, int causal, int window, int lo, int hi) {
    return (key < S) & (!causal | (key <= q)) & ((window <= 0) | (key > q - window)) & (key >= lo) & (key < hi);
}
template <bool EXPL>
LRP_DEVICE float lrp_ds(float s_raw, float p, float dp, float Dq, float scale, float eps_mask, float eps_qk) {
    if constexpr (!EXPL) return p * (dp - Dq);
    else {
        const float s2 = s_raw * scale;
        return p * (dp - Dq) * scale * (s2 * s_raw) * __builtin_amdgcn_rcpf((s2 + eps_mask) * (2.f * s_raw + eps_qk));
    }
}

struct IvWave { int lo_min, hi_max, lo_max, hi_min; };
LRP_DEVICE int wave_min(int v) {
#pragma unroll
    for (int off = 32; off > 0; off >>= 1) v = min(v, __shfl_xor(v, off, 64));
    return v;
}
LRP_DEVICE int wave_max(int v) {
#pragma unroll
    for (int off = 32; off > 0; off >>= 1) v = max(v, __shfl_xor(v, off, 64));
    return v;
}
LRP_DEVICE IvWave iv_wave(int lo, int hi, bool in_range, int wave, int* sh) {
    const bool sees = in_range && hi > lo;
    IvWave w;
    w.lo_min = wave_min(sees ? lo : 0x7fffffff);
    w.hi_max = wave_max(sees ? hi : 0);
    w.lo_max = wave_max(in_range ? lo : 0);
    w.hi_min = wave_min(in_range ? hi : 0x7fffffff);
    sh[2 * wave] = w.lo_min;
    sh[2 * wave + 1] = w.hi_max;
    return w;
}
// ... 41 lines not shown
```

### lrp-explains-transformers_amd/csrc/common.hpp

```cpp
#pragma once
#include <hip/hip_runtime.h>
#include <stdint.h>
#include "../../include/lrp_hip.h"

typedef __bf16 bf16_t;
typedef __attribute__((ext_vector_type(8))) __bf16 bf16x8;
typedef __attribute__((ext_vector_type(4))) __bf16 bf16x4;
typedef __attribute__((ext_vector_type(2))) __bf16 bf16x2;
typedef __attribute__((ext_vector_type(4))) float f32x4;
typedef __attribute__((ext_vector_type(2))) float f32x2;
typedef __attribute__((ext_vector_type(16))) float f32x16;
typedef __attribute__((ext_vector_type(4))) uint32_t u32x4;
typedef __attribute__((ext_vector_type(2))) uint32_t u32x2;

#define LRP_DEVICE __device__ __forceinline__

extern thread_local int g_lrp_last_hip_error;

#include <atomic>
static inline void lrp_set_max_lds_once(std::atomic<uint64_t>& done, const void* kern, size_t bytes) {
    int dev = 0;
    (void)hipGetDevice(&dev);
    const uint64_t bit = 1ull << (dev & 63);
    if (done.load(std::memory_order_acquire) & bit) return;
// ... 75 lines not shown
}
LRP_DEVICE float block_sum(float x, float* red) {
    x = wave_sum(x);
    const int w = threadIdx.x >> 6, nw = blockDim.x >> 6;
    __syncthreads();
    if ((threadIdx.x & 63) == 0) red[w] = x;
    __syncthreads();
    float t = 0.f;
    for (int i = 0; i < nw; ++i) t += red[i];
    return t;
}
LRP_DEVICE float block_max(float x, float* red) {
    x = wave_max(x);
    const int w = threadIdx.x >> 6, nw = blockDim.x >> 6;
    __syncthreads();
    if ((threadIdx.x & 63) == 0) red[w] = x;
    __syncthreads();
    float t = red[0];
    for (int i = 1; i < nw; ++i) t = fmaxf(t, red[i]);
    return t;
}

LRP_DEVICE float eps_ratio(float z, float c, float eps) {
    return (eps == 0.f) ? (1.f / c) : z / (c * z + eps);
}

LRP_DEVICE float act_apply(float x, int act) {
    if (act == LRP_ACT_SILU) return x / (1.f + __expf(-x));
    if (act == LRP_ACT_GELU_TANH) {
        const float k0 = 0.7978845608028654f, k1 = 0.044715f;
        return 0.5f * x * (1.f + tanhf(k0 * (x + k1 * x * x * x)));
    }
    if (act == LRP_ACT_TANH) return tanhf(x);
    return 0.5f * x * (1.f + erff(x * 0.7071067811865476f));
}

template <bool FAST> LRP_DEVICE float fdiv_t(float a, float b) {
    if constexpr (FAST) return a * __builtin_amdgcn_rcpf(b);
    else return a / b;
}
template <bool FAST> LRP_DEVICE float fdiv_small_t(float a, float b) {
    if constexpr (FAST) {
        const float sc = (fabsf(b) < 1.17549435e-38f) ? 16777216.f : 1.f;
        return a * (__builtin_amdgcn_rcpf(b * sc) * sc);
    } else return a / b;
}
template <bool FAST> LRP_DEVICE float eps_ratio_t(float z, float c, float eps) {
    return (eps == 0.f) ? fdiv_t<FAST>(1.f, c) : fdiv_t<FAST>(z, c * z + eps);
}
template <bool FAST> LRP_DEVICE float act_apply_t(float x, int act) {
    if constexpr (FAST) {
        if (act == LRP_ACT_SILU) return x * __builtin_amdgcn_rcpf(1.f + __expf(-x));
        if (act == LRP_ACT_GELU_TANH) {
            const float k0 = 0.7978845608028654f, k1 = 0.044715f;
            return x * __builtin_amdgcn_rcpf(1.f + __expf(-2.f * k0 * (x + k1 * x * x * x)));
        }
    }
    return act_apply(x, act);
}

template <bool LEAN, int ACT_CT = -1>
LRP_DEVICE void gated_bwd_pair_bf16(float g, float u, float gmh, float eps_g, float eps_lin, int act, float& ag, float& au) {
    const int a_ = ACT_CT >= 0 ? ACT_CT : act;
    const float y = (float)(bf16_t)act_apply_t<true>(g, a_);
    const float den = g + eps_g;
    if constexpr (LEAN) {
        const float q = y * __builtin_amdgcn_rcpf(den);
        ag = gmh * u * ((den == 0.f) ? 0.f : q);
        au = gmh * y;
    } else {
        ag = (den == 0.f) ? 0.f : gmh * u * fdiv_small_t<true>(y, den);
        au = gmh * y * eps_ratio_t<true>(u, 1.f, eps_lin);
    }
}

template <bool LEAN, int ACT_CT>
LRP_DEVICE void gated_coef(float g, float u, float eps_g, float eps_lin, float& m, float& cg, float& cu) {
    const float y = act_apply_t<true>(g, ACT_CT);
    m = y * u;
    const float den = g + eps_g, hy = 0.5f * y;
    if constexpr (LEAN) {
        const float q = hy * __builtin_amdgcn_rcpf(den);
        cg = (den == 0.f) ? 0.f : u * q;
        cu = hy;
    } else {
        cg = (den == 0.f) ? 0.f : u * fdiv_small_t<true>(hy, den);
        cu = hy * eps_ratio_t<true>(u, 1.f, eps_lin);
    }
}
LRP_DEVICE float bf16_lo(uint32_t w) { return __builtin_bit_cast(float, w << 16); }
LRP_DEVICE float bf16_hi(uint32_t w) { return __builtin_bit_cast(float, w & 0xffff0000u); }

LRP_DEVICE void mx_decode8(uint32_t word, uint32_t E, bf16_t* out) {
    const float sc = __builtin_bit_cast(float, E << 23);
    bf16x2 v0 = __builtin_amdgcn_cvt_scalef32_pk_bf16_fp4(word, sc, 0), v1 = __builtin_amdgcn_cvt_scalef32_pk_bf16_fp4(word, sc, 1);
    bf16x2 v2 = __builtin_amdgcn_cvt_scalef32_pk_bf16_fp4(word, sc, 2), v3 = __builtin_amdgcn_cvt_scalef32_pk_bf16_fp4(word, sc, 3);
    out[0] = v0[0]; out[1] = v0[1]; out[2] = v1[0]; out[3] = v1[1]; out[4] = v2[0]; out[5] = v2[1]; out[6] = v3[0]; out[7] = v3[1];
}
LRP_DEVICE void mx_decode8(uint32_t word, uint32_t E, float* out) {
    const float sc = __builtin_bit_cast(float, E << 23);
    f32x2 v0 = __builtin_amdgcn_cvt_scalef32_pk_f32_fp4(word, sc, 0), v1 = __builtin_amdgcn_cvt_scalef32_pk_f32_fp4(word, sc, 1);
    f32x2 v2 = __builtin_amdgcn_cvt_scalef32_pk_f32_fp4(word, sc, 2), v3 = __builtin_amdgcn_cvt_scalef32_pk_f32_fp4(word, sc, 3);
    out[0] = v0[0]; out[1] = v0[1]; out[2] = v1[0]; out[3] = v1[1]; out[4] = v2[0]; out[5] = v2[1]; out[6] = v3[0]; out[7] = v3[1];
}

template <typename T> struct Mma16;
template <> struct Mma16<bf16_t> {
    typedef bf16x8 frag;
    static LRP_DEVICE f32x4 mma(frag a, frag b, f32x4 c) {
        return __builtin_amdgcn_mfma_f32_16x16x32_bf16(a, b, c, 0, 0, 0);
    }
};
template <> struct Mma16<float> {
    typedef f32x4 frag;
    static LRP_DEVICE f32x4 mma(frag a, frag b, f32x4 c) {
        c = __builtin_amdgcn_mfma_f32_16x16x4f32(a[0], b[0], c, 0, 0, 0);
        c = __builtin_amdgcn_mfma_f32_16x16x4f32(a[1], b[1], c, 0, 0, 0);
        c = __builtin_amdgcn_mfma_f32_16x16x4f32(a[2], b[2], c, 0, 0, 0);
        c = __builtin_amdgcn_mfma_f32_16x16x4f32(a[3], b[3], c, 0, 0, 0);
        return c;
    }
};

LRP_DEVICE void grouped_tile(int id, int tiles_m, int tiles_n, int& tm, int& tn) {
    constexpr int GROUP_M = 8;
    const int per_group = GROUP_M * tiles_n;
    const int group = id / per_group;
    const int first_m = group * GROUP_M;
    const int gsz = (tiles_m - first_m) < GROUP_M ? (tiles_m - first_m) : GROUP_M;
    const int in_group = id - group * per_group;
    tm = first_m + in_group % gsz;
    tn = in_group / gsz;
}

LRP_DEVICE int xcd_remap(int bid, int nwg) {
    const int q = nwg >> 3, r = nwg & 7, xcd = bid & 7, loc = bid >> 3;
    const int base = (xcd < r) ? xcd * (q + 1) : r * (q + 1) + (xcd - r) * q;
    return base + loc;
}

struct AttnCall {
    const void *q, *k, *v, *gho;
    const float* lse;
    const float* D;
    int B, S, Hq, Hkv, d;
    int64_t ldq, ldk, ldv, ldg, ldt;
    float scale, eps_mask, eps_qk;
    int causal, window, q_begin;
    const int *row_lo, *row_hi;
    hipStream_t st;
    void* o;  float* lse_out;  int64_t ldo;  const void* v_t;
    void* dq;  int64_t lddq;  const void* k_t;
    const void* ofw;  float* Dout;  const float *cos_t, *sin_t;
    void *dk, *dv;  int64_t lddk, lddv;  const void *q_t, *gho_t;
};

int lrp_attn32_fwd(const AttnCall& c);
int lrp_attn32_dq(const AttnCall& c);
int lrp_attn32_dkv(const AttnCall& c);

static inline int xcd_group_grid(int ngroups, int per_group) { return ((ngroups + 7) / 8) * 8 * per_group; }

struct PPEpi {
    bf16_t* c2;
    int64_t ldc2;
    const bf16_t* gu;
    int64_t ldgu;
    float eps_g, eps_lin;
    int act;
    const float* rs;
    const bf16_t* res;
    int64_t ldres;
    float* ssq;
    int64_t ldssq;
    const float* cos;
    const float* sin;
    int seq;
    int rope_cols;
};

struct PPFused {
    const bf16_t* A;
    const bf16_t* B;
    bf16_t* C;
    const bf16_t* bias;
    int M, N, K;
    int64_t lda, ldb, ldc;
    int nn, epi;
    PPEpi ep;
};

int lrp_launch_gemm_pp(const void* A, const void* B, void* C, const void* bias, int M, int N, int K, int64_t lda, int64_t ldb,
                       int64_t ldc, int out_dtype, int nn, int splits, int kt_per_split, int64_t slab_stride, hipStream_t st);
int lrp_launch_gemm_pp_fused(const PPFused& f, hipStream_t st);
```

### lrp-explains-transformers_amd/engine.py

```python
import collections
import math
import operator

import torch

from . import ops
from .engine_cp import cp_layer_bwd, cp_request

EXPLICIT = dict(lin=1e-8, add=1e-8, qk=1e-8, mask=1e-8, pv=1e-6, rope=1e-8, act=None)
EFFICIENT = dict(lin=0.0, add=0.0, qk=0.0, mask=0.0, pv=0.0, rope=0.0, act=1e-10)


_STATIC_ROPE = ("default", "linear", "llama3", "yarn")


def rope_kind(hf_cfg):
    rp = getattr(hf_cfg, "rope_parameters", None)
    if isinstance(rp, dict):
        return rp.get("rope_type", rp.get("type", "default"))
    rs = getattr(hf_cfg, "rope_scaling", None)
    if rs is None:
        return "default"
    if isinstance(rs, dict) and (rs.get("rope_type") or rs.get("type")):
        return rs.get("rope_type") or rs.get("type")
# ... 33 lines not shown
    m = model.model
    W = dict(embed=m.embed_tokens.weight.detach(), norm=m.norm.weight.detach(), lm_head=model.lm_head.weight.detach(),
             layers=[])
    for L in m.layers:
        a, mlp = L.self_attn, L.mlp
        W["layers"].append(dict(ln1=L.input_layernorm.weight.detach(), ln2=L.post_attention_layernorm.weight.detach(),
                                wq=a.q_proj.weight.detach(), wk=a.k_proj.weight.detach(), wv=a.v_proj.weight.detach(),
                                wo=a.o_proj.weight.detach(), wg=mlp.gate_proj.weight.detach(),
                                wu=mlp.up_proj.weight.detach(), wd=mlp.down_proj.weight.detach()))
    return config_from_hf(model.config), W


PITCH_PAD = True


def pitch_pad(cols, elem_size):
    nbytes = cols * elem_size
    if not PITCH_PAD:
        return 0
    return 128 // elem_size if (nbytes >= 16384 and nbytes % 4096 == 0) else 0


def weight_pitch_pad(cols, elem_size, rows=0):
    nbytes = cols * elem_size
    if not PITCH_PAD or nbytes % 1024 != 0 or rows * nbytes < (32 << 20):
        return 0
    return 256 // elem_size



def fused_layout(H, I, nq, nk, d, dtype):
    es = dtype.itemsize
    nqkv = (nq + 2 * nk) * d
    return dict(Wqkv=H + weight_pitch_pad(H, es, nqkv), Wgu=H + weight_pitch_pad(H, es, 2 * I), Wd=I + pitch_pad(I, es),
                m=I + pitch_pad(I, es), Agu=2 * I + pitch_pad(2 * I, es), Aqkv=nqkv + (64 if PITCH_PAD and (nqkv * es) % 4096 == 0 else 0))


def fold_rows(dst, srcs, ln):
    lnf = ln.detach().to(device=dst.device, dtype=torch.float32)
    r0 = 0
    for w in srcs:
        for b0 in range(0, w.shape[0], 4096):
            blk = w[b0: b0 + 4096].detach()
            dst[r0 + b0: r0 + b0 + blk.shape[0]].copy_((blk.float() * lnf).to(dst.dtype))
        r0 += w.shape[0]
    return dst


FusedOk = collections.namedtuple("FusedOk", "coef norm prep full")


def fused_layer_ok(M, W, meta, dtype, cache):
    key = (M, PITCH_PAD, repr(ops.NORM_FUSION), ops.GATED_FUSION, ops.PREP_FUSION, ops.ROPE_BWD_FUSION)
    hit = cache.get(key)
    if hit is None:
        nq, nk, d, _, act, _ = meta
        H, I, nqkv = W["wo"].shape[0], W["wd"].shape[1], (nq + 2 * nk) * d
        pt = fused_layout(H, I, nq, nk, d, dtype)
        ldo, ldqkv, ldgu, ldd = (W[k].stride(0) for k in ("wo", "wqkv", "wgu", "wd"))
        coef = ops.gated_coef_ok(M, I, H, H, ldgu, H, ldd, act, dtype)
        norm = coef and all(ops.norm_fused_ok(*a, dtype) for a in (
            (M, H, nq * d, nq * d, ldo, False),
            (M, H, I, pt["m"], ldd, False),
            (M, nqkv, H, H, ldqkv, False),
            (M, 2 * I, H, H, ldgu, False),
            (M, H, nqkv, pt["Aqkv"], ldqkv, True),
            (M, H, 2 * I, pt["Agu"], ldgu, True)))
        prep = ops.attn_dq_d_ok(dtype, d) and ops.norm_fused_ok(M, nq * d, H, H, ldo, True, dtype)
        full = (norm and prep and all(ops.norm_fusion_part(p) for p in ("fwd", "bwd_gu", "bwd_qkv")) and ops.ROPE_BWD_FUSION
                and d in (64, 128))
        hit = cache[key] = FusedOk(bool(coef), bool(norm), bool(prep), bool(full))
    return hit


def fused_qkv_fwd(h, rstd1, Wqkv, cos, sin, S, meta, alloc, explicit=False, bias=None, qk_norm=None):
    nq, nk, d = meta[:3]
    M, nqk = h.shape[0], (nq + nk) * d
    qkv = alloc("qkv", M, (nq + 2 * nk) * d, 0, h.dtype)
    if qk_norm is not None:
        if bias is None:
            ops.gemm_nt_rs(h, Wqkv, rstd1, qkv)
        else:
            ops.gemm_nt_rs_bias(h, Wqkv, rstd1, bias, qkv)
        qkr = alloc("qkr", M, nqk, 0, h.dtype)
        rstd_q, rstd_k = alloc("rstd_q", 1, M * nq, 0, torch.float32)[0], alloc("rstd_k", 1, M * nk, 0, torch.float32)[0]
        ops.qk_norm_rope_fwd(qkv, qk_norm[0], qk_norm[1], qkr[:, : nq * d], qkr[:, nq * d:], rstd_q, rstd_k, cos, sin, S, nq, nk, d, meta[3])
        return qkv, qkr, rstd_q, rstd_k
    if bias is not None:
        if not explicit and ops.gemm_nt_rs_bias_rope_ok(h, Wqkv, qkv, S, nqk, d):
            return qkv, ops.gemm_nt_rs_bias_rope(h, Wqkv, rstd1, bias, cos, sin, qkv, S, nqk, d)[:, :nqk]
        ops.gemm_nt_rs_bias(h, Wqkv, rstd1, bias, qkv)
        return qkv, ops.rope_fwd(qkv, alloc("qkr", M, nqk, 0, h.dtype), cos, sin, S, nq + nk, d)
    if not explicit and ops.gemm_nt_rs_rope_ok(h, Wqkv, qkv, S, nqk, d):
        return qkv, ops.gemm_nt_rs_rope(h, Wqkv, rstd1, cos, sin, qkv, S, nqk, d)[:, :nqk]
    ops.gemm_nt_rs(h, Wqkv, rstd1, qkv)
    return qkv, ops.rope_fwd(qkv, alloc("qkr", M, nqk, 0, h.dtype), cos, sin, S, nq + nk, d)


def fused_attn_fwd(h, qkv, qkr, W, B, S, meta, alloc, row_iv=None, explicit=False):
    nq, nk, d, rms_eps, _, scale = meta
    M, H, dt = B * S, h.shape[1], h.dtype
    new = lambda tag, cols: alloc(tag, M, cols, 0, dt)
    v = qkv[:, (nq + nk) * d:]
    v_t = ops.transpose_heads(v, B, S, nk, d) if ops.attn_needs_transposed(v, d) else None
    st = dict(o=new("o", nq * d), lse=alloc("lse", B * nq, S, 0, torch.float32).view(B, nq, S))
    ops.attn_fwd(qkr[:, : nq * d], qkr[:, nq * d:], v, v_t, st["o"], st["lse"], B, S, nq, nk, d, scale, True, 0, row_iv=row_iv)
    ssq = alloc("ssq", H // 64, M, 0, torch.float32)
    st.update(h1=new("h1", H), a=new("a", H) if explicit else None)
    ops.gemm_res_ssq(st["o"], W["wo"], h, st["h1"], ssq, raw=st["a"])
    st["rstd2"] = ops.rms_rstd(ssq, M, H, rms_eps, alloc("rstd2", 1, M, 0, torch.float32)[0])
    return st, ssq


def fused_layer_fwd(h, rstd1, qkv, qkr, W, cos, sin, B, S, meta, alloc, row_iv=None, explicit=False, eps=(EFFICIENT["act"], EFFICIENT["lin"]),
                    chain=True):
    nq, nk, d, rms_eps, act, scale = meta
    M, H, I, dt = B * S, h.shape[1], W["wd"].shape[1], h.dtype
    new = lambda tag, cols, pitch=None: alloc(tag, M, cols, (pitch or cols) - cols, dt)
    vec = lambda tag: alloc(tag, 1, M, 0, torch.float32)[0]
    st, ssq = fused_attn_fwd(h, qkv, qkr, W, B, S, meta, alloc, row_iv, explicit)
    pt = fused_layout(H, I, nq, nk, d, dt)
    st["gu"], m = ops.gemm_gated_fwd_coef(st["h1"], W["wgu"], new("gu", 2 * I), new("m", I, pt["m"]), *eps, act, rs=st["rstd2"])
    st["m"] = m
    if chain:
        st["h_out"], st["dn"] = new("h_out", H), new("dn", H) if explicit else None
        ops.gemm_res_ssq(m, W["wd"], st["h1"], st["h_out"], ssq, raw=st["dn"])
        st["rstd_out"] = ops.rms_rstd(ssq, M, H, rms_eps, vec("rstd_out"))
    else:
        st["dn"] = ops.linear_fwd(m, W["wd"], out=new("dn", H))
    return st


def fused_layer_bwd(G, st, W, cos, sin, B, S, meta, alloc, row_iv=None, qk_norm=None, heads=None, attn_map=None, weights=None):
    nq, nk, d = meta[:3]
    M, H, I, dt = B * S, G.shape[1], W["wd"].shape[1], G.dtype
    pt = fused_layout(H, I, nq, nk, d, dt)
    new = lambda tag, cols, pitch=None: alloc(tag, M, cols, (pitch or cols) - cols, dt)
    Agu = ops.gemm_gated_bwd_coef(G, W["wd"], st["gu"], new("Agu", 2 * I, pt["Agu"]))
    if weights is not None:
        weights("down", G, st["m"], W["wd"])
        weights("gate_up", Agu, st["h1"], W["wgu"], rs=st["rstd2"])
    Gs1 = ops.gemm_nn_rs_res(Agu, W["wgu"], st["rstd2"], G, new("Gs1", H))
    return fused_attn_bwd(Gs1, st, W, cos, sin, B, S, meta, alloc, row_iv, qk_norm, heads, attn_map, weights)


def fused_attn_bwd(Gs1, st, W, cos, sin, B, S, meta, alloc, row_iv=None, qk_norm=None, heads=None, attn_map=None, weights=None):
    nq, nk, d, _, _, scale = meta
    M, H, dt, nqk, nqkv = B * S, Gs1.shape[1], Gs1.dtype, (nq + nk) * d, (nq + 2 * nk) * d
    pt = fused_layout(H, 0, nq, nk, d, dt)
    new = lambda tag, cols, pitch=None: alloc(tag, M, cols, (pitch or cols) - cols, dt)
    Gho = ops.gemm_nn_rs(Gs1, W["wo"], alloc("half", 1, M, 0, torch.float32)[0], new("Gho", nq * d))
    q, k, v = st["qkr"][:, : nq * d], st["qkr"][:, nq * d:], st["qkv"][:, nqk:]
    D = alloc("D", B * nq, S, 0, torch.float32).view(B, nq, S)
    Aqkv, dk_h, dv_h = new("Aqkv", nqkv, pt["Aqkv"]), new("dk_h", nq * d), new("dv_h", nq * d)
    if heads is not None:
        heads("out", st["o"], Gho, scale=2.0)
    if weights is not None:
        weights("o", Gs1, st["o"], W["wo"])
    if attn_map is not None:
        attn_map(q, k, v, Gho, st["lse"], 2.0, row_iv)
    if qk_norm is not None:
        dq = ops.attn_bwd_dq_d(q, k, v, Gho, st["o"], st["lse"], D, new("dq", nq * d), B, S, nq, nk, d, scale, row_iv=row_iv)
        ops.attn_bwd_dkv(q, k, v, None, Gho, None, st["lse"], D, dk_h, dv_h, B, S, nq, nk, d, scale, 0.0, 0.0, row_iv=row_iv)
        if heads is not None:
            heads("q", q, dq)
            heads("k", k, dk_h, nq // nk)
            heads("v", v, dv_h, nq // nk)
        ops.qkv_bwd_pack(dq, dk_h, dv_h, qk_norm[0], qk_norm[1], st["rstd_q"], st["rstd_k"], cos, sin, Aqkv, S, nq, nk, d)
        if weights is not None:
            weights("qkv", Aqkv, st["h"], W["wqkv"], rs=st["rstd1"])
        return ops.gemm_nn_rs_res(Aqkv, W["wqkv"], st["rstd1"], Gs1, new("Gh", H))
    ops.attn_bwd_dq_d(q, k, v, Gho, st["o"], st["lse"], D, Aqkv[:, : nq * d], B, S, nq, nk, d, scale, row_iv=row_iv, rope=(cos, sin))
    ops.attn_bwd_dkv(q, k, v, None, Gho, None, st["lse"], D, dk_h, dv_h, B, S, nq, nk, d, scale, 0.0, 0.0, row_iv=row_iv)
    if heads is not None:
        heads("q", q, Aqkv[:, : nq * d], rope=(cos, sin))
        heads("k", k, dk_h, nq // nk)
        heads("v", v, dv_h, nq // nk)
    ops.gqa_reduce_rope(dk_h, Aqkv[:, nq * d: nqk], M, S, nk, nq // nk, d, cos, sin)
    ops.gqa_reduce(dv_h, Aqkv[:, nqk:], M, nk, nq // nk, d)
    if weights is not None:
        weights("qkv", Aqkv, st["h"], W["wqkv"], rs=st["rstd1"])
    return ops.gemm_nn_rs_res(Aqkv, W["wqkv"], st["rstd1"], Gs1, new("Gh", H))


FUSED_SCRATCH = frozenset(("ssq", "m", "half", "Agu", "Gs1", "Gho", "D", "Aqkv", "dk_h", "dv_h", "dq"))



def pack_flat(top, layer, n_layers, dtype, device, align=64):
    up = lambda n: (n + align - 1) // align * align
    stored = lambda shape, pitch: (*shape[:-1], pitch or shape[-1])
    specs = [top] + (list(layer) if isinstance(layer, (list, tuple)) else [layer] * n_layers)
    flat = torch.empty(sum(up(math.prod(stored(*e))) for spec in specs for e in spec.values()), device=device, dtype=dtype)
    views, o = [], 0
    for spec in specs:
        views.append({})
        for name, (shape, pitch) in spec.items():
            full = stored(shape, pitch)
            views[-1][name] = flat[o: o + math.prod(full)].view(full)[..., : shape[-1]]
            o += up(math.prod(full))
    return flat, views[0], views[1:]


def put_rows(dst, *srcs):
    o = 0
    for t in srcs:
        dst[o: o + t.shape[0]].copy_(t.to(device=dst.device, dtype=dst.dtype, non_blocking=True))
        o += t.shape[0]
    return dst


def put_gate_up(dst, wg, wu):
    return ops.interleave_gate_up(wg.to(device=dst.device, dtype=dst.dtype), wu.to(device=dst.device, dtype=dst.dtype), out=dst)


WEIGHT_FORMATS = (None, "mxfp4")
MX_MATRICES = ("wqkv", "wo", "wgu", "wd")


def weight_format_request(weight_format, cfg):
    if weight_format not in WEIGHT_FORMATS:
        raise ValueError(f"weight_format must be one of {WEIGHT_FORMATS}, got {weight_format!r}")
    if weight_format == "mxfp4":
        for name, K in (("hidden", cfg["hidden"]), ("n_heads * head_dim", cfg["n_heads"] * cfg["head_dim"]), ("inter", cfg["inter"])):
            if K % ops.MX_BLOCK:
                raise ValueError(f"weight_format='mxfp4': {name} = {K} is not a multiple of {ops.MX_BLOCK} (one scale per {ops.MX_BLOCK} "
                                 "elements along a Linear's contraction dimension)")
    return weight_format


def quant_layout(layer):
    rest = {k: v for k, v in layer.items() if k not in MX_MATRICES}
    lin = {k: layer[k] for k in MX_MATRICES}
    q = {}
    for k, ((N, K), _) in lin.items():
        q[k + "_c"] = ((N, K // 2), None)
        q[k + "_s"] = ((N, K // ops.MX_BLOCK), (K // ops.MX_BLOCK + 3) // 4 * 4)
    return rest, lin, q


def rope_tables(inv_freq, attention_scaling, max_seq, dtype, device):
    fr = torch.arange(max_seq, dtype=torch.float32)[:, None] * inv_freq.float().cpu()[None, :]
    emb = torch.cat((fr, fr), dim=-1)
    return ((emb.cos() * attention_scaling).to(dtype).to(torch.float32).to(device).contiguous(),
            (emb.sin() * attention_scaling).to(dtype).to(torch.float32).to(device).contiguous())


class Arena:

    def __init__(self, device, dtype):
        self.device, self.dtype, self.buf = device, dtype, {}
        self.gen = 0

    def get(self, tag, shape, dtype, zero=False, pad=0):
        full = tuple(shape[:-1]) + (shape[-1] + pad,) if pad else tuple(shape)
        n = math.prod(full)
        t = self.buf.get((tag, dtype))
        if t is None or t.numel() < n:
            if t is not None:
                self.gen += 1
            t = torch.empty(max(n, 1), device=self.device, dtype=dtype)
            self.buf[(tag, dtype)] = t
        v = t[:n].view(*full)
        if zero:
            v.zero_()
        return v[..., : shape[-1]] if pad else v

    def new(self, tag, *shape):
        return self.get(tag, shape, self.dtype)

    def f32(self, tag, *shape):
        return self.get(tag, shape, torch.float32)

    def zeros(self, tag, *shape):
        return self.get(tag, shape, self.dtype, zero=True)

    def wide(self, tag, rows, cols):
        return self.get(tag, (rows, cols), self.dtype, pad=pitch_pad(cols, self.dtype.itemsize))

    def nbytes(self):
        return sum(t.numel() * t.element_size() for t in self.buf.values())


def explain_inputs(input_ids, inputs_embeds, lengths, target, vocab, max_seq, dtype, device, seed=None):
    B, S = input_ids.shape if inputs_embeds is None else inputs_embeds.shape[:2]
    if S > max_seq:
        raise ValueError(f"sequence length {S} exceeds max_seq={max_seq}")
    row_iv = None
    if lengths is not None:
        lens = torch.as_tensor(lengths, device=device).to(torch.int32).reshape(B)
        if int(lens.min()) < 1 or int(lens.max()) > S:
            raise ValueError("lengths must lie in [1, S]")
        i = torch.arange(S, device=device, dtype=torch.int32)
        first = (S - lens)[:, None]
        lo = first.expand(B, S).contiguous()
        hi = torch.where(i[None] >= first, (i + 1)[None].expand(B, S), torch.zeros_like(lo)).contiguous()
        row_iv = (lo, hi)
    idx = None
    if target is not None:
        tgt = torch.as_tensor(target).reshape(-1).cpu().long()
        if tgt.numel() != B or int(tgt.min()) < 0 or int(tgt.max()) >= vocab:
            raise ValueError(f"target must hold {B} vocabulary indices in [0, {vocab})")
        idx = tgt.to(device=device, dtype=torch.int32).contiguous()
    if seed is not None:
        if target is not None:
            raise ValueError("pass either target or seed, not both")
        if tuple(seed.shape) != (B, vocab):
            raise ValueError(f"seed must have shape ({B}, {vocab}), got {tuple(seed.shape)}")
    emb = None if inputs_embeds is None else inputs_embeds.to(device=device, dtype=dtype).reshape(B * S, -1).contiguous()
    return B, S, emb, row_iv, idx


def generate_request(input_ids, inputs_embeds, max_new_tokens, lengths, eos_token_id, pad_token_id, vocab, max_seq):
    if inputs_embeds is not None or input_ids is None:
        raise ValueError("generate takes input_ids: every new token is fed back through the embedding table, inputs_embeds have no ids to continue")
    try:
        ids = torch.as_tensor(input_ids).cpu()
    except (TypeError, ValueError, RuntimeError):
        raise ValueError(f"input_ids must be an integer tensor [B, S], got {input_ids!r}") from None
    if ids.dim() != 2 or ids.shape[0] < 1 or ids.shape[1] < 1 or ids.is_floating_point() or ids.dtype == torch.bool:
        raise ValueError(f"input_ids must be integers of shape [B, S], got {tuple(ids.shape)} {ids.dtype}")
    ids = ids.long()
    B, S = ids.shape
    if int(ids.min()) < 0 or int(ids.max()) >= vocab:
        raise ValueError(f"input_ids must hold vocabulary indices in [0, {vocab})")
    if isinstance(max_new_tokens, bool) or not isinstance(max_new_tokens, int) or max_new_tokens < 1:
        raise ValueError(f"max_new_tokens must be an integer >= 1, got {max_new_tokens!r}")
    if S + max_new_tokens > max_seq:
        raise ValueError(f"S + max_new_tokens = {S + max_new_tokens} exceeds max_seq={max_seq} (the RoPE tables and the cache end there)")
    if lengths is None:
        lens = torch.full((B,), S, dtype=torch.long)
    else:
        try:
            lens = torch.as_tensor(lengths).cpu()
        except (TypeError, ValueError, RuntimeError):
            raise ValueError(f"lengths must be {B} integers, got {lengths!r}") from None
        if lens.numel() != B or lens.is_floating_point() or lens.dtype == torch.bool or int(lens.min()) < 1 or int(lens.max()) > S:
            raise ValueError(f"lengths must be {B} integers in [1, {S}]")
# ... 1152 lines not shown
```

### lrp-explains-transformers_amd/ops.py

```python
import torch

from ._lib import lib, check, F32, BF16, ACT

_DT = {torch.float32: F32, torch.bfloat16: BF16}


def dt(t):
    try:
        return _DT[t.dtype]
    except KeyError:
        raise TypeError(f"lrp_hip supports float32 and bfloat16 tensors, got {t.dtype}") from None


def p(t):
    if t is None:
        return None
    if not t.is_cuda:
        raise RuntimeError("lrp_hip kernels need device tensors (no CPU fallback)")
    return t.data_ptr()


def stream():
    return torch.cuda.current_stream().cuda_stream

# ... 1092 lines not shown
        if main is not None and (out is None or out.stride(1) == 1):
            if out is None:
                out = torch.empty(M, N, device=x2.device, dtype=odt)
            bias = aux(bias, x2, N)
            gemm_nt_2d(x2, W[:main], out[:, :main], None if bias is None else bias[:main])
            gemm_skinny(x2, W[main:], out[:, main:], nn=False, bias=None if bias is None else bias[main:])
            return out
    if splitk_ok(M, N, K) and gemm_nn_ok(x2, W):
        if out is None:
            out = torch.empty(M, N, device=x2.device, dtype=odt)
        return gemm_skinny(x2, W, out, nn=False, bias=bias)
    if smallm_ok(M, W, x2):
        return linear_smallm_fwd(x2, W, bias, out=out, out_dtype=odt)
    if out is not None and x2.stride(1) == 1 and W.stride(1) == 1 and x2.dtype == W.dtype and x2.stride(0) % epc(x2) == 0:
        return gemm_nt_2d(x2, W, out, bias)
    z = gemm_nt(x2, W, bias, out_dtype=odt)
    if out is not None:
        out.copy_(z)
        return out
    return z


STREAM_DGRAD = True


def linear_stream_dgrad_ok(s2, W):
    if not STREAM_DGRAD or s2.dtype != torch.bfloat16 or W.dtype != torch.bfloat16 or s2.dim() != 2 or W.dim() != 2:
        return False
    if s2.stride(1) != 1 or W.stride(1) != 1 or s2.data_ptr() % 16 or W.data_ptr() % 16:
        return False
    return bool(lib.lrp_linear_stream_dgrad_ok(s2.shape[0], W.shape[0], W.shape[1], s2.stride(0), W.stride(0)))


def linear_stream_dgrad(s2, W, out=None, out_dtype=None, z=None, eps=0.0, relevance_in=False):
    M, N = s2.shape
    Kout = W.shape[1]
    same(s2, W, z)
    if z is not None and (z.stride(1) != 1 or tuple(z.shape) != (M, N)):
        raise ValueError("linear_stream_dgrad: z must be [M, N] with contiguous rows")
    if z is not None and eps == 0.0:
        if relevance_in:
            raise ValueError("linear_stream_dgrad: a relevance operand needs eps != 0 (s / (z + 0) has no defined value at z = 0)")
        z = None
    if out is None:
        out = torch.empty(M, Kout, device=s2.device, dtype=out_dtype or s2.dtype)
    need = lib.lrp_linear_stream_dgrad_ws(M, N, Kout)
    ws = workspace(need, s2) if need else None
    ntk = lib.lrp_linear_stream_dgrad_tickets(M, N, Kout) if STREAM_DGRAD_INKERNEL_REDUCE else 0
    check(lib.lrp_linear_stream_dgrad_tk(p(s2), p(z), p(W), p(out), M, N, Kout, s2.stride(0), z.stride(0) if z is not None else 0, W.stride(0),
                                         out.stride(0), eps, int(relevance_in), dt(s2), _DT[out.dtype], p(ws), p(tickets(ntk, s2) if ntk else None),
                                         stream()), "lrp_linear_stream_dgrad_tk")
    return out


def linear_dgrad(s2, W, out=None, out_dtype=None):
    M, N = s2.shape
    K = W.shape[1]
    odt = out_dtype or (out.dtype if out is not None else W.dtype)
    if M <= 32 and linear_stream_dgrad_ok(s2, W) and (out is None or (out.stride(1) == 1 and out.dtype in _DT)):
        return linear_stream_dgrad(s2, W, out=out, out_dtype=odt)
    nn = gemm_nn_ok(s2, W)
    if (M <= 2 or (M <= SMALLM_MAX and not nn)) and N >= 16 and smallm_ok(M, W) and s2.stride(1) == 1 and s2.dtype == W.dtype:
        return linear_smallm_dgrad(s2, W, out=out, out_dtype=odt)
    if nn and M > SKINNY_MAX:
        main = tail_split_cols(M, K, N)
        if main is not None and (out is None or out.stride(1) == 1) and W.data_ptr() % 16 == 0:
            if out is None:
                out = torch.empty(M, K, device=s2.device, dtype=odt)
            gemm_nn_2d(s2, W[:, :main], out[:, :main])
            gemm_skinny(s2, W[:, main:], out[:, main:], nn=True)
            return out
    if nn:
        split = splitk_ok(M, K, N)
        if split or ((M + 255) // 256) * ((K + 255) // 256) >= 190:
            if out is None:
                out = torch.empty(M, K, device=s2.device, dtype=odt)
            return gemm_skinny(s2, W, out, nn=True) if split else gemm_nn_2d(s2, W, out)
    wt = weight_t(W)
    if out is not None and s2.stride(1) == 1 and s2.dtype == wt.dtype and s2.stride(0) % epc(s2) == 0:
        return gemm_nt_2d(s2, wt, out)
    c = gemm_nt(s2, wt, out_dtype=odt)
    if out is not None:
        out.copy_(c)
        return out
    return c


def clear_weight_cache(*weights):
    for w in weights:
        _WT.pop(w.untyped_storage()._cdata, None)


def pad_to(n, m):
    return (n + m - 1) // m * m


def transpose_heads(x, B, S, H, d, out=None):
    ldt = pad_to(S, 64)
    if out is None:
        out = torch.zeros(B, H, d, ldt, device=x.device, dtype=x.dtype)
    check(lib.lrp_transpose_heads(p(x), p(out), B, S, H, d, x.stride(0), out.stride(2), dt(x), stream()), "lrp_transpose_heads")
    return out


def _iv(row_iv, B, S):
    if row_iv is None:
        return 0, 0
    lo, hi = row_iv
    for t in (lo, hi):
        if t.dtype != torch.int32 or not t.is_contiguous() or t.numel() != B * S or not t.is_cuda:
            raise ValueError("row intervals must be contiguous int32 CUDA tensors of B*S elements")
    return lo.data_ptr(), hi.data_ptr()


def attn_needs_transposed(t, d):
    return bool(lib.lrp_attn_needs_transposed(dt(t), d))


def attn_fwd(q, k, v, v_t, o, lse, B, S, Hq, Hkv, d, scale, causal=True, window=0, q_begin=0, row_iv=None):
    same(q, k, v, v_t, o)
    f32(lse)
    check(lib.lrp_attn_fwd(p(q), p(k), p(v), p(v_t), p(o), p(lse), B, S, Hq, Hkv, d, q.stride(0), k.stride(0), v.stride(0),
                           v_t.stride(2) if v_t is not None else 0, o.stride(0), scale, int(causal), window, q_begin,
                           *_iv(row_iv, B, S), dt(q), stream()), "lrp_attn_fwd")
    return o, lse


def attn_bwd_prep(Go, o, Gho, D, B, S, Hq, d, eps_pv, factor=0.5):
    same(Go, o, Gho)
    f32(D)
    check(lib.lrp_attn_bwd_prep(p(Go), p(o), p(Gho), p(D), B, S, Hq, d, Go.stride(0), o.stride(0), Gho.stride(0), eps_pv,
                                factor, dt(Go), stream()), "lrp_attn_bwd_prep")
    return Gho, D


def attn_bwd_dq(q, k, v, k_t, Gho, lse, D, dq, B, S, Hq, Hkv, d, scale, eps_mask, eps_qk, causal=True, window=0, q_begin=0,
                row_iv=None):
    same(q, k, v, k_t, Gho, dq)
    f32(lse, D)
    check(lib.lrp_attn_bwd_dq(p(q), p(k), p(v), p(k_t), p(Gho), p(lse), p(D), p(dq), B, S, Hq, Hkv, d, q.stride(0),
                              k.stride(0), v.stride(0), k_t.stride(2) if k_t is not None else 0, Gho.stride(0), dq.stride(0),
                              scale, eps_mask, eps_qk,
                              int(causal), window, q_begin, *_iv(row_iv, B, S), dt(q), stream()), "lrp_attn_bwd_dq")
    return dq


PREP_FUSION = True


def attn_dq_d_ok(dtype, d):
    return bool(PREP_FUSION and dtype in _DT and lib.lrp_attn_bwd_dq_d_ok(_DT[dtype], d))


def attn_bwd_dq_d(q, k, v, Gho, o, lse, D, dq, B, S, Hq, Hkv, d, scale, causal=True, window=0, row_iv=None, rope=None):
    same(q, k, v, Gho, o, dq)
    f32(lse, D)
    cs, sn = rope if rope is not None else (None, None)
    f32(cs, sn)
    check(lib.lrp_attn_bwd_dq_d(p(q), p(k), p(v), p(Gho), p(o), p(lse), p(D), p(dq), B, S, Hq, Hkv, d, q.stride(0), k.stride(0), v.stride(0),
                                Gho.stride(0), o.stride(0), dq.stride(0), scale, int(causal), window, *_iv(row_iv, B, S), p(cs), p(sn), dt(q),
                                stream()), "lrp_attn_bwd_dq_d")
    return dq


ROPE_BWD_FUSION = True


def gqa_reduce_rope(x, out, rows, seq, Hkv, rep, d, cos, sin):
    f32(cos, sin)
    check(lib.lrp_gqa_reduce_rope(p(x), p(out), rows, seq, Hkv, rep, d, x.stride(0), out.stride(0), p(cos), p(sin), dt(x), stream()),
          "lrp_gqa_reduce_rope")
    return out


def attn_bwd_dkv(q, k, v, q_t, Gho, Gho_t, lse, D, dk_h, dv_h, B, S, Hq, Hkv, d, scale, eps_mask, eps_qk, causal=True,
                 window=0, q_begin=0, row_iv=None):
    same(q, k, v, q_t, Gho, Gho_t, dk_h, dv_h)
    f32(lse, D)
    check(lib.lrp_attn_bwd_dkv(p(q), p(k), p(v), p(q_t), p(Gho), p(Gho_t), p(lse), p(D), p(dk_h), p(dv_h), B, S, Hq, Hkv, d,
                               q.stride(0), k.stride(0), v.stride(0), q_t.stride(2) if q_t is not None else 0, Gho.stride(0),
                               dk_h.stride(0),
                               dv_h.stride(0), scale, eps_mask, eps_qk, int(causal), window, q_begin, *_iv(row_iv, B, S), dt(q), stream()),
          "lrp_attn_bwd_dkv")
    return dk_h, dv_h


def attn_bwd_dv_ok(dtype, d):
    return bool(dtype in _DT and lib.lrp_attn_bwd_dv_ok(_DT[dtype], d))


def attn_bwd_dv(q, k, G, lse, dv, B, S, Hq, Hkv, d, scale, q_begin=0, row_iv=None, q_t=None, G_t=None):
    same(q, k, G, dv, q_t, G_t)
    f32(lse)
    check(lib.lrp_attn_bwd_dv(p(q), p(k), p(G), p(G_t), p(lse), p(dv), B, S, Hq, Hkv, d, q.stride(0), k.stride(0), G.stride(0),
                              G_t.stride(2) if G_t is not None else 0, dv.stride(0), scale, q_begin, *_iv(row_iv, B, S), dt(q), stream()),
          "lrp_attn_bwd_dv")
    return dv


def gqa_reduce(x, out, rows, Hkv, rep, d):
    check(lib.lrp_gqa_reduce(p(x), p(out), rows, Hkv, rep, d, x.stride(0), out.stride(0), dt(x), stream()), "lrp_gqa_reduce")
    return out


ATTN_DECODE_SLAB = int(lib.lrp_attn_decode_slab())


def _decode_rows(name, t, what, rows, cols, ref=None):
    if t.dim() != 2 or t.shape[0] != rows or t.shape[1] != cols or t.stride(1) != 1:
        raise ValueError(f"{name}: {what} {tuple(t.shape)} must be [{rows}, {cols}] with contiguous rows")
    if ref is not None:
        same(ref, t)


def _decode_cache(name, kc, vc, B, cols, ref):
    for what, t in (("kc", kc), ("vc", vc)):
        if t.dim() != 3 or t.shape[0] != B or t.shape[2] != cols or t.shape[1] < 1 or t.stride(2) != 1 or t.shape != kc.shape \
                or t.stride() != kc.stride() or (B > 1 and t.stride(0) != t.shape[1] * t.stride(1)):
            raise ValueError(f"{name}: {what} {tuple(t.shape)} / strides {t.stride()} must be [{B}, cap, {cols}] with contiguous rows, batch stride "
                             "cap * row pitch, kc and vc alike")
    same(ref, kc, vc)
    return int(kc.shape[1]), int(kc.stride(1))


def _decode_pos(name, pos, ref):
    if pos.dtype != torch.int32 or pos.numel() != 1 or pos.device != ref.device:
        raise TypeError(f"{name}: pos must be an int32 tensor of one element on {ref.device} (the step's column, read on the device)")


def decode_rope_append(qk, v, cos, sin, pos, q_rot, kc, vc, nq, nk, d):
    B = qk.shape[0]
    pq = p(qk)
    _decode_rows("decode_rope_append", qk, "qk", B, (nq + nk) * d)
    _decode_rows("decode_rope_append", v, "v", B, nk * d, qk)
    _decode_rows("decode_rope_append", q_rot, "q_rot", B, nq * d, qk)
    cap, ldc = _decode_cache("decode_rope_append", kc, vc, B, nk * d, qk)
    _decode_pos("decode_rope_append", pos, qk)
    f32(cos, sin)
    if cos.dim() != 2 or cos.shape[1] != d or cos.shape != sin.shape or not cos.is_contiguous() or not sin.is_contiguous():
        raise ValueError(f"decode_rope_append: cos / sin must be contiguous [rows, {d}] tables")
    ld = lambda t: t.stride(0) if B > 1 else max(t.stride(0), t.shape[1])
    check(lib.lrp_decode_rope_append(pq, ld(qk), p(v), ld(v), p(cos), p(sin), cos.shape[0], p(pos), p(q_rot), ld(q_rot), p(kc), p(vc), ldc, B, cap,
                                     nq, nk, d, dt(qk), stream()), "lrp_decode_rope_append")
    return q_rot


def decode_qknorm_rope_append(qk, v, wq, wk, eps, cos, sin, pos, q_rot, kc, vc, nq, nk, d, w_offset=0.0):
    B = qk.shape[0]
    pq = p(qk)
    _decode_rows("decode_qknorm_rope_append", qk, "qk", B, (nq + nk) * d)
    _decode_rows("decode_qknorm_rope_append", v, "v", B, nk * d, qk)
    _decode_rows("decode_qknorm_rope_append", q_rot, "q_rot", B, nq * d, qk)
    cap, ldc = _decode_cache("decode_qknorm_rope_append", kc, vc, B, nk * d, qk)
    _decode_pos("decode_qknorm_rope_append", pos, qk)
    f32(cos, sin)
    if cos.dim() != 2 or cos.shape[1] != d or cos.shape != sin.shape or not cos.is_contiguous() or not sin.is_contiguous():
        raise ValueError(f"decode_qknorm_rope_append: cos / sin must be contiguous [rows, {d}] tables")
    same(qk, wq, wk)
    if wq.numel() != d or wk.numel() != d or not wq.is_contiguous() or not wk.is_contiguous():
        raise ValueError(f"decode_qknorm_rope_append: wq / wk must be contiguous [{d}] norm weights")
    ld = lambda t: t.stride(0) if B > 1 else max(t.stride(0), t.shape[1])
    check(lib.lrp_decode_qknorm_rope_append(pq, ld(qk), p(v), ld(v), p(wq), p(wk), float(eps), float(w_offset), p(cos), p(sin), cos.shape[0],
                                            p(pos), p(q_rot), ld(q_rot), p(kc), p(vc), ldc, B, cap, nq, nk, d, dt(qk), stream()),
          "lrp_decode_qknorm_rope_append")
    return q_rot


def attn_decode_ws(B, Hq, d, cap):
    n = int(lib.lrp_attn_decode_ws(B, Hq, d, cap))
    if n < 0:
        raise ValueError(f"attn_decode: no kernel for B = {B}, Hq = {Hq}, d = {d}, cap = {cap} (d a multiple of 8, at most 256)")
    return n


def attn_decode(q, kc, vc, lo, pos, Hq, Hkv, d, scale, out=None, ws=None):
    B = q.shape[0]
    pq = p(q)
    _decode_rows("attn_decode", q, "q", B, Hq * d)
    cap, ldc = _decode_cache("attn_decode", kc, vc, B, Hkv * d, q)
    _decode_pos("attn_decode", pos, q)
    if lo.dtype != torch.int32 or lo.numel() != B or not lo.is_contiguous() or lo.device != q.device:
        raise TypeError(f"attn_decode: lo must be a contiguous int32 [{B}] tensor on {q.device}")
    if out is None:
        out = torch.empty(B, Hq * d, device=q.device, dtype=q.dtype)
    _decode_rows("attn_decode", out, "out", B, Hq * d, q)
    if B == 0:
        return out
    need = attn_decode_ws(B, Hq, d, cap)
    if ws is None:
        ws = workspace(need, q)
    elif ws.dtype != torch.uint8 or ws.numel() < need or not ws.is_contiguous() or ws.device != q.device:
        raise ValueError(f"attn_decode: ws must be a contiguous uint8 tensor of >= {need} bytes on {q.device}")
    ld = lambda t: t.stride(0) if B > 1 else max(t.stride(0), t.shape[1])
    check(lib.lrp_attn_decode(pq, ld(q), p(kc), p(vc), ldc, p(lo), p(pos), p(out), ld(out), p(ws), ws.numel(), B, cap, Hq, Hkv, d, float(scale),
                              dt(q), stream()), "lrp_attn_decode")
    return out


class MoePlan:

    def __init__(self, idx, E):
        if idx.dim() != 2:
            raise ValueError(f"lrp_moe_plan: top_k_index must be [T, k], got {tuple(idx.shape)}")
        self.T, self.k, self.E = int(idx.shape[0]), int(idx.shape[1]), int(E)
        n = lib.lrp_moe_plan_ints(self.T, self.k, self.E)
        if n < 0:
            check(int(n), "lrp_moe_plan_ints")
        p(idx)
        idx = idx.to(torch.int64).contiguous()
        self.buf = torch.empty(int(n), device=idx.device, dtype=torch.int32)
        check(lib.lrp_moe_plan(p(idx), p(self.buf), self.T, self.k, self.E, stream()), "lrp_moe_plan")

    @property
    def rows(self):
        return self.T * self.k

    def views(self):
        E, R, b = self.E, self.rows, self.buf
        return b[:E], b[E:2 * E + 1], b[3 * E + 2:3 * E + 2 + R], b[3 * E + 2 + R:3 * E + 2 + 2 * R]


class MoeQuantWeight:

    def __init__(self, w, codes=None, scales=None):
        if not w.is_cuda:
            raise RuntimeError("MoeQuantWeight: lrp_hip kernels need device tensors (no CPU fallback)")
        if w.dim() != 3 or not w.is_contiguous() or w.shape[2] % (4 * MX_BLOCK):
            raise ValueError(f"MoeQuantWeight: an expert tensor is a contiguous [E, N, K] with K % {4 * MX_BLOCK} == 0, got {tuple(w.shape)}")
        E, N, K = w.shape
        if codes is None:
            codes = torch.empty(E, N, K // 2, device=w.device, dtype=torch.uint8)
# ... 309 lines not shown
```

Before: 22.01.

## Seed dkv MFMA accumulators with precomputed row constants instead of zero

The dq kernel now also writes a per-row constant buffer holding -lse/scale and -D. The dkv kernel uses it to start its score and dP MFMA accumulators at these offsets rather than at zero, so the later per-element subtraction of lse and D is folded into the matrix multiply's initial value. The row constants are read from LDS early and prefetched for the next sub-tile. This removes per-element work in the hot loop at the cost of an extra scratch buffer, new wait-count bookkeeping, and a path limited to bf16 with head dims 64, 96 or 128.

Result: no change. 22.04, median of 6 (+0.1%).

```diff
diff --git a/include/lrp_hip.h b/include/lrp_hip.h
--- a/include/lrp_hip.h
+++ b/include/lrp_hip.h
@@ -232,4 +232,5 @@
 #include "lrp_hip_mxfp4_stream.h"
 #include "lrp_hip_sample.h"
 #include "lrp_hip_attn_cp.h"
+#include "lrp_hip_attn_rc.h"
 #endif
diff --git a/include/lrp_hip_attn_rc.h b/include/lrp_hip_attn_rc.h
--- /dev/null
+++ b/include/lrp_hip_attn_rc.h
@@ -0,0 +1,20 @@
+#ifndef LRP_HIP_ATTN_RC_H
+#define LRP_HIP_ATTN_RC_H
+#include <stdint.h>
+#ifdef __cplusplus
+extern "C" {
+#endif
+
+int lrp_attn_bwd_dq_d_rc(const void* q, const void* k, const void* v, const void* Gho, const void* o, const float* lse, float* D, void* dq,
+                         int B, int S, int Hq, int Hkv, int d, int64_t ldq, int64_t ldk, int64_t ldv, int64_t ldgho, int64_t ldo, int64_t lddq,
+                         float scale, int causal, int window, const int* row_lo, const int* row_hi, const float* cos_t, const float* sin_t,
+                         int dtype, void* stream, float* rc);
+int lrp_attn_bwd_dkv_rc(const void* q, const void* k, const void* v, const void* q_t, const void* Gho, const void* Gho_t, const float* lse,
+                        const float* D, void* dk_h, void* dv_h, int B, int S, int Hq, int Hkv, int d, int64_t ldq, int64_t ldk, int64_t ldv,
+                        int64_t ldt, int64_t ldgho, int64_t lddk, int64_t lddv, float scale, float eps_mask, float eps_qk, int causal,
+                        int window, int q_begin, const int* row_lo, const int* row_hi, int dtype, void* stream, const float* rc);
+
+#ifdef __cplusplus
+}
+#endif
+#endif
diff --git a/lrp-explains-transformers_amd/csrc/attention.hip b/lrp-explains-transformers_amd/csrc/attention.hip
--- a/lrp-explains-transformers_amd/csrc/attention.hip
+++ b/lrp-explains-transformers_amd/csrc/attention.hip
@@ -1048,10 +1048,10 @@
 
 extern "C" int lrp_attn_bwd_dq_d_ok(int dtype, int d) { return (use_attn32(dtype, d) && d != 256) ? 1 : 0; }
 
-extern "C" int lrp_attn_bwd_dq_d(const void* q, const void* k, const void* v, const void* Gho, const void* o, const float* lse, float* D,
-                                 void* dq, int B, int S, int Hq, int Hkv, int d, int64_t ldq, int64_t ldk, int64_t ldv, int64_t ldgho,
-                                 int64_t ldo, int64_t lddq, float scale, int causal, int window, const int* row_lo, const int* row_hi,
-                                 const float* cos_t, const float* sin_t, int dtype, void* stream) {
+static int attn_bwd_dq_d_call(const void* q, const void* k, const void* v, const void* Gho, const void* o, const float* lse, float* D,
+                              void* dq, int B, int S, int Hq, int Hkv, int d, int64_t ldq, int64_t ldk, int64_t ldv, int64_t ldgho,
+                              int64_t ldo, int64_t lddq, float scale, int causal, int window, const int* row_lo, const int* row_hi,
+                              const float* cos_t, const float* sin_t, int dtype, void* stream, float* rcon) {
     if ((cos_t == nullptr) != (sin_t == nullptr)) return LRP_EINVAL;
     if (cos_t && d != 64 && d != 128) return LRP_ESHAPE;
     if ((row_lo == nullptr) != (row_hi == nullptr)) return LRP_EINVAL;
@@ -1068,8 +1068,28 @@
     c.ldq = ldq; c.ldk = ldk; c.ldv = ldv; c.ldg = ldgho;
     c.scale = scale; c.causal = causal; c.window = window;
     c.row_lo = row_lo; c.row_hi = row_hi; c.st = (hipStream_t)stream;
-    c.dq = dq; c.lddq = lddq; c.ofw = o; c.ldo = ldo; c.Dout = D; c.cos_t = cos_t; c.sin_t = sin_t;
+    c.dq = dq; c.lddq = lddq; c.ofw = o; c.ldo = ldo; c.Dout = D; c.cos_t = cos_t; c.sin_t = sin_t; c.rc = rcon;
     return lrp_attn32_dq(c);
+}
+
+extern "C" int lrp_attn_bwd_dq_d(const void* q, const void* k, const void* v, const void* Gho, const void* o, const float* lse, float* D,
+                                 void* dq, int B, int S, int Hq, int Hkv, int d, int64_t ldq, int64_t ldk, int64_t ldv, int64_t ldgho,
+                                 int64_t ldo, int64_t lddq, float scale, int causal, int window, const int* row_lo, const int* row_hi,
+                                 const float* cos_t, const float* sin_t, int dtype, void* stream) {
+    return attn_bwd_dq_d_call(q, k, v, Gho, o, lse, D, dq, B, S, Hq, Hkv, d, ldq, ldk, ldv, ldgho, ldo, lddq, scale, causal, window, row_lo, row_hi,
+                              cos_t, sin_t, dtype, stream, nullptr);
+}
+
+static inline bool attn_rc_served(int dtype, int d) { return dtype == LRP_BF16 && (d == 64 || d == 96 || d == 128); }
+
+extern "C" int lrp_attn_bwd_dq_d_rc(const void* q, const void* k, const void* v, const void* Gho, const void* o, const float* lse, float* D,
+                                    void* dq, int B, int S, int Hq, int Hkv, int d, int64_t ldq, int64_t ldk, int64_t ldv, int64_t ldgho,
+                                    int64_t ldo, int64_t lddq, float scale, int causal, int window, const int* row_lo, const int* row_hi,
+                                    const float* cos_t, const float* sin_t, int dtype, void* stream, float* rc) {
+    if (!rc || !attn_rc_served(dtype, d)) return LRP_EINVAL;
+    if (reinterpret_cast<uintptr_t>(rc) & 3) return LRP_EALIGN;
+    return attn_bwd_dq_d_call(q, k, v, Gho, o, lse, D, dq, B, S, Hq, Hkv, d, ldq, ldk, ldv, ldgho, ldo, lddq, scale, causal, window, row_lo, row_hi,
+                              cos_t, sin_t, dtype, stream, rc);
 }
 
 template <typename T>
@@ -1093,11 +1113,11 @@
     return lrp_check_launch();
 }
 
-extern "C" int lrp_attn_bwd_dkv(const void* q, const void* k, const void* v, const void* q_t, const void* Gho,
-                                const void* Gho_t, const float* lse, const float* D, void* dk_h, void* dv_h, int B, int S,
-                                int Hq, int Hkv, int d, int64_t ldq, int64_t ldk, int64_t ldv, int64_t ldt, int64_t ldgho,
-                                int64_t lddk, int64_t lddv, float scale, float eps_mask, float eps_qk, int causal, int window,
-                                int q_begin, const int* row_lo, const int* row_hi, int dtype, void* stream) {
+static int attn_bwd_dkv_call(const void* q, const void* k, const void* v, const void* q_t, const void* Gho,
+                             const void* Gho_t, const float* lse, const float* D, void* dk_h, void* dv_h, int B, int S,
+                             int Hq, int Hkv, int d, int64_t ldq, int64_t ldk, int64_t ldv, int64_t ldt, int64_t ldgho,
+                             int64_t lddk, int64_t lddv, float scale, float eps_mask, float eps_qk, int causal, int window,
+                             int q_begin, const int* row_lo, const int* row_hi, int dtype, void* stream, const float* rcon) {
     if ((row_lo == nullptr) != (row_hi == nullptr)) return LRP_EINVAL;
     if (!q || !k || !v || !Gho || !lse || !D || !dk_h || !dv_h) return LRP_EINVAL;
     int rc = attn_common_check(B, S, Hq, Hkv, d, dtype, scale);
@@ -1117,9 +1137,29 @@
     c.ldq = ldq; c.ldk = ldk; c.ldv = ldv; c.ldg = ldgho; c.ldt = ldt;
     c.scale = scale; c.eps_mask = eps_mask; c.eps_qk = eps_qk; c.causal = causal; c.window = window; c.q_begin = q_begin;
     c.row_lo = row_lo; c.row_hi = row_hi; c.st = (hipStream_t)stream;
-    c.dk = dk_h; c.dv = dv_h; c.lddk = lddk; c.lddv = lddv; c.q_t = q_t; c.gho_t = Gho_t;
+    c.dk = dk_h; c.dv = dv_h; c.lddk = lddk; c.lddv = lddv; c.q_t = q_t; c.gho_t = Gho_t; c.rc = const_cast<float*>(rcon);
     if (a32) return lrp_attn32_dkv(c);
     return dtype == LRP_F32 ? attn_dkv_t<float>(c) : attn_dkv_t<bf16_t>(c);
+}
+
+extern "C" int lrp_attn_bwd_dkv(const void* q, const void* k, const void* v, const void* q_t, const void* Gho,
+                                const void* Gho_t, const float* lse, const float* D, void* dk_h, void* dv_h, int B, int S,
+                                int Hq, int Hkv, int d, int64_t ldq, int64_t ldk, int64_t ldv, int64_t ldt, int64_t ldgho,
+                                int64_t lddk, int64_t lddv, float scale, float eps_mask, float eps_qk, int causal, int window,
+                                int q_begin, const int* row_lo, const int* row_hi, int dtype, void* stream) {
+    return attn_bwd_dkv_call(q, k, v, q_t, Gho, Gho_t, lse, D, dk_h, dv_h, B, S, Hq, Hkv, d, ldq, ldk, ldv, ldt, ldgho, lddk, lddv, scale, eps_mask,
+                             eps_qk, causal, window, q_begin, row_lo, row_hi, dtype, stream, nullptr);
+}
+
+extern "C" int lrp_attn_bwd_dkv_rc(const void* q, const void* k, const void* v, const void* q_t, const void* Gho,
+                                   const void* Gho_t, const float* lse, const float* D, void* dk_h, void* dv_h, int B, int S,
+                                   int Hq, int Hkv, int d, int64_t ldq, int64_t ldk, int64_t ldv, int64_t ldt, int64_t ldgho,
+                                   int64_t lddk, int64_t lddv, float scale, float eps_mask, float eps_qk, int causal, int window,
+                                   int q_begin, const int* row_lo, const int* row_hi, int dtype, void* stream, const float* rc) {
+    if (!rc || !attn_rc_served(dtype, d) || eps_mask != 0.f || eps_qk != 0.f) return LRP_EINVAL;
+    if (reinterpret_cast<uintptr_t>(rc) & 3) return LRP_EALIGN;
+    return attn_bwd_dkv_call(q, k, v, q_t, Gho, Gho_t, lse, D, dk_h, dv_h, B, S, Hq, Hkv, d, ldq, ldk, ldv, ldt, ldgho, lddk, lddv, scale, eps_mask,
+                             eps_qk, causal, window, q_begin, row_lo, row_hi, dtype, stream, rc);
 }
 
 extern "C" int lrp_transpose_heads(const void* x, void* xt, int B, int S, int H, int d, int64_t ldx, int64_t ldt,
diff --git a/lrp-explains-transformers_amd/csrc/attention32.hip b/lrp-explains-transformers_amd/csrc/attention32.hip
--- a/lrp-explains-transformers_amd/csrc/attention32.hip
+++ b/lrp-explains-transformers_amd/csrc/attention32.hip
@@ -162,13 +162,14 @@
     if (hi == 0 && qi < S) lse[((int64_t)b * Hq + h) * S + qi] = m_run * scale + __logf(l_run);
 }
 
-template <bool EXPL, int DH>
+template <bool EXPL, int DH, bool RC = false>
 __global__ __launch_bounds__(NWQ * 64, 2) void dq_kernel(
     const bf16_t* __restrict__ q, const bf16_t* __restrict__ k, const bf16_t* __restrict__ v, const bf16_t* __restrict__ gho,
     const float* __restrict__ lse, const float* __restrict__ Dd, bf16_t* __restrict__ dq, int S, int Hq, int Hkv, int64_t ldq,
     int64_t ldk, int64_t ldv, int64_t ldg, int64_t lddq, float scale, float eps_mask, float eps_qk, int causal, int window,
     int B, int q_begin, const int* __restrict__ row_lo, const int* __restrict__ row_hi, const bf16_t* __restrict__ ofw, int64_t ldo,
-    float* __restrict__ Dout, const float* __restrict__ rope_cos, const float* __restrict__ rope_sin) {
+    float* __restrict__ Dout, const float* __restrict__ rope_cos, const float* __restrict__ rope_sin, float* __restrict__ rc) {
+    static_assert(!(RC && EXPL), "the explicit placement needs the raw score");
     constexpr int BQ = NWQ * 32, STAGE = 2 * TILE, NK = DH / 16, ND32 = DH / 32;
     extern __shared__ __attribute__((aligned(16))) char smem[];
     const int lane = threadIdx.x & 63, l31 = lane & 31, hi = lane >> 5;
@@ -186,7 +187,8 @@
     bf16x8 qf[NK], gf[NK];
     load_row_frags<DH>(qf, q + (int64_t)b * S * ldq + (int64_t)h * DH, ldq, qi, S, hi);
     load_row_frags<DH>(gf, gho + (int64_t)b * S * ldg + (int64_t)h * DH, ldg, qi, S, hi);
-    const float lse2 = ((qi < S) ? lse[((int64_t)b * Hq + h) * S + qi] : 0.f) * LRP_LOG2E;
+    const float lse_q = (qi < S) ? lse[((int64_t)b * Hq + h) * S + qi] : 0.f;
+    const float lse2 = lse_q * LRP_LOG2E;
     float Dq;
     if (ofw != nullptr) {
         bf16x8 of[NK];
@@ -200,6 +202,12 @@
         Dq = sd;
         if (hi == 0 && qi < S) Dout[((int64_t)b * Hq + h) * S + qi] = sd;
     } else Dq = (qi < S) ? Dd[((int64_t)b * Hq + h) * S + qi] : 0.f;
+    if constexpr (RC) {
+        if (hi == 0 && qi < S) {
+            rc[((int64_t)b * Hq + h) * S + qi] = -(lse_q / scale);
+            rc[((int64_t)(B + b) * Hq + h) * S + qi] = -Dq;
+        }
+    }
     int ivlo = 0, ivhi = S;
     if (row_lo != nullptr && qi < S) { ivlo = row_lo[(int64_t)b * S + qi]; ivhi = row_hi[(int64_t)b * S + qi]; }
     f32x16 acc[ND32];
@@ -351,12 +359,13 @@
 #endif
 }
 
-template <bool EXPL, int DH, bool IV>
+template <bool EXPL, int DH, bool IV, bool RC = false>
 __global__ __launch_bounds__(512, 2) void dkv_kernel(
     const bf16_t* __restrict__ q, const bf16_t* __restrict__ k, const bf16_t* __restrict__ v, const bf16_t* __restrict__ gho,
     const float* __restrict__ lse, const float* __restrict__ Dd, bf16_t* __restrict__ dk, bf16_t* __restrict__ dv, int S, int Hq,
     int Hkv, int64_t ldq, int64_t ldk, int64_t ldv, int64_t ldg, int64_t lddk, int64_t lddv, float scale, float eps_mask,
     float eps_qk, int causal, int window, int B, int q_begin, const int* __restrict__ row_lo, const int* __restrict__ row_hi) {
+    static_assert(!(RC && EXPL), "the explicit placement needs the raw score");
     constexpr int BK = NW * 32, STAGE = 2 * TILE + 512, VROWS = 32 * KP, NK = DH / 16, ND32 = DH / 32;
     extern __shared__ __attribute__((aligned(16))) char smem[];
     const int lane = threadIdx.x & 63, l31 = lane & 31, hi = lane >> 5;
@@ -427,11 +436,19 @@
     const uint32_t tl_start = tl_prev;
 #endif
     int cur = 0;
+    f32x4 cs[4], cd[4];
+#define A32_RC_READ(SO_)                                                                  \
+    A32_RD128(cs[0], ast, (SO_)); A32_RD128(cd[0], ast, (SO_) + 256);                     \
+    A32_RD128(cs[1], ast, (SO_) + 32); A32_RD128(cd[1], ast, (SO_) + 32 + 256);           \
+    A32_RD128(cs[2], ast, (SO_) + 64); A32_RD128(cd[2], ast, (SO_) + 64 + 256);           \
+    A32_RD128(cs[3], ast, (SO_) + 96); A32_RD128(cd[3], ast, (SO_) + 96 + 256)
     for (int qt0 = qbeg; qt0 < qend; qt0 += CT) {
+        if constexpr (RC) { A32_RC_READ(0); }
         if (qt0 + CT < qend) stage(qt0 + CT, cur ^ 1);
         A32_TS(0);
         sfor<0, 2>([&](auto qbc) {
             constexpr int qb = decltype(qbc)::value, QO = qb * 32 * KP, SO = qb * 128;
+            constexpr int PF = (RC && qb == 0) ? 8 : 0;
             const int qq0 = qt0 + qb * 32;
             bool live = !((causal && qq0 + 31 < kw) || qq0 >= S);
             bool iv_mask = false;
@@ -441,9 +458,16 @@
                 if (t1_ <= kw || t0_ >= kw + 32) live = false;
                 iv_mask = !(t2_ <= kw && t3_ >= kw + 32);
             }
-            if (!live) return;
-            f32x16 st = zero16(), dp = zero16();
+            if (!live) {
+                if constexpr (PF != 0) { A32_RC_READ(128); }
+                return;
+            }
+            f32x16 st, dp;
             f32x4 sl[2], sd[2];
+            if constexpr (!RC) {
+                st = zero16();
+                dp = zero16();
+            }
             constexpr int PD = 2, RS = PD + 1;
             bf16x8 fq[RS], fg[RS], fv[RS];
             static_assert(PD < NK, "read-ahead deeper than the contraction");
@@ -458,12 +482,17 @@
             sfor<0, NK>([&](auto ksc) {
                 constexpr int ks = decltype(ksc)::value, cu = ks % RS, nx = (ks + PD) % RS;
                 constexpr int ahead = (ks + PD < NK ? PD : NK - 1 - ks);
+                if constexpr (RC && ks == 0) {
+                    A32_WAIT(6, "+v"(cs[0]), "+v"(cs[1]), "+v"(cs[2]), "+v"(cs[3]), "+v"(cd[0]), "+v"(cd[1]), "+v"(cd[2]), "+v"(cd[3]));
+                    st = join16(cs);
+                    dp = join16(cd);
+                }
                 if constexpr (ks + PD < NK) {
                     const uint32_t aq = frag_addr<ks + PD>(arm0), av = frag_addr<ks + PD>(avw0);
                     A32_RD128(fq[nx], aq, QO); A32_RD128(fg[nx], aq, QO + TILE); A32_RD128(fv[nx], av, 0);
                 }
-                if constexpr (ks == NK - 2) { A32_RD128(sl[0], ast, SO); A32_RD128(sd[0], ast, SO + 256); }
-                constexpr int nw = 3 * ahead + (ks >= NK - 2 ? 2 : 0);
+                if constexpr (!RC && ks == NK - 2) { A32_RD128(sl[0], ast, SO); A32_RD128(sd[0], ast, SO + 256); }
+                constexpr int nw = 3 * ahead + (!RC && ks >= NK - 2 ? 2 : 0);
                 static_assert(nw <= 14, "lgkmcnt is a 4-bit counter");
                 asm volatile("s_waitcnt lgkmcnt(%[n])" : "+v"(fq[cu]), "+v"(fg[cu]), "+v"(fv[cu]) : [n] "n"(nw));
                 st = mfma32(fq[cu], kf[ks], st);
@@ -476,6 +505,13 @@
     A32_RDTR(tg[slot][0], atr[dbb][0], QO + TILE + (jj) * 16 * KP); A32_RDTR(tg[slot][1], atr[dbb][1], QO + TILE + (jj) * 16 * KP); \
     A32_RDTR(tq[slot][0], atr[dbb][0], QO + (jj) * 16 * KP); A32_RDTR(tq[slot][1], atr[dbb][1], QO + (jj) * 16 * KP)
 #define A32_TIE(sl_) "+v"(tg[sl_][0]), "+v"(tg[sl_][1]), "+v"(tq[sl_][0]), "+v"(tq[sl_][1])
+#define A32_WAITN(n, ...) asm volatile("s_waitcnt lgkmcnt(%[n_])" : __VA_ARGS__ : [n_] "n"(n))
+#define A32_FIRST                                                                                      \
+    if constexpr (RC) asm volatile("s_waitcnt lgkmcnt(4)" : A32_TIE(sl_))
+#define A32_FIRST_PF                                                                                   \
+    if constexpr (RC) A32_WAITN(4 + PF, A32_TIE(sl_))
+#define A32_NEXT_RC                                                                                    \
+    if constexpr (PF != 0) { A32_RC_READ(128); }
 #define A32_DKV_STEP(g, wait_stmt)                                                                     \
     {                                                                                                  \
         constexpr int j_ = (g) / ND32, db_ = (g) % ND32, sl_ = (g)&1;                                  \
@@ -488,7 +524,8 @@
             bf16x8 pf[2], df[2];
             auto elementwise = [&](auto ic) {
                 constexpr int i = decltype(ic)::value, cu = i & 1, nx = cu ^ 1;
-                if constexpr (i == 0) {
+                if constexpr (RC) {
+                } else if constexpr (i == 0) {
                     A32_RD128(sl[nx], ast, SO + 32); A32_RD128(sd[nx], ast, SO + 32 + 256);
                     A32_WAIT(6, "+v"(sl[cu]), "+v"(sd[cu]));
                 } else if constexpr (i == 1) {
@@ -504,7 +541,10 @@
                 }
                 float pe[4];
 #pragma unroll
-                for (int e = 0; e < 4; ++e) pe[e] = fast_exp2(__builtin_fmaf(st[4 * i + e], c1, -(sl[cu][e] * LRP_LOG2E)));
+                for (int e = 0; e < 4; ++e) {
+                    if constexpr (RC) pe[e] = fast_exp2(st[4 * i + e] * c1);
+                    else pe[e] = fast_exp2(__builtin_fmaf(st[4 * i + e], c1, -(sl[cu][e] * LRP_LOG2E)));
+                }
                 if (masked) {
 #pragma unroll
                     for (int e = 0; e < 4; ++e) {
@@ -518,7 +558,8 @@
                 for (int e = 0; e < 4; ++e) {
                     const int r = 4 * i + e;
                     pf[i >> 1][4 * (i & 1) + e] = (bf16_t)pe[e];
-                    df[i >> 1][4 * (i & 1) + e] = (bf16_t)lrp_ds<EXPL>(st[r], pe[e], dp[r], sd[cu][e], scale, eps_mask, eps_qk);
+                    if constexpr (RC) df[i >> 1][4 * (i & 1) + e] = (bf16_t)(pe[e] * dp[r]);
+                    else df[i >> 1][4 * (i & 1) + e] = (bf16_t)lrp_ds<EXPL>(st[r], pe[e], dp[r], sd[cu][e], scale, eps_mask, eps_qk);
                 }
                 A32_FENCE();
             };
@@ -529,7 +570,7 @@
             if constexpr (ND32 == 4) {
                 A32_TS(2);
                 A32_TRG(1, 0, 1);
-                A32_DKV_STEP(0, (void)0);
+                A32_DKV_STEP(0, A32_FIRST);
                 A32_TRG(0, 0, 2);
                 A32_DKV_STEP(1, A32_WAIT(4, A32_TIE(1)));
                 A32_TRG(1, 0, 3);
@@ -541,16 +582,17 @@
                 elementwise(IC<3>{});
                 A32_TS(2);
                 A32_TRG(1, 1, 1);
-                A32_DKV_STEP(4, (void)0);
+                A32_NEXT_RC;
+                A32_DKV_STEP(4, A32_FIRST_PF);
                 A32_TRG(0, 1, 2);
-                A32_DKV_STEP(5, A32_WAIT(4, A32_TIE(1)));
+                A32_DKV_STEP(5, A32_WAITN(4 + PF, A32_TIE(1)));
                 A32_TRG(1, 1, 3);
                 A32_DKV_STEP(6, A32_WAIT(4, A32_TIE(0)));
                 A32_DKV_STEP(7, A32_WAIT(0, A32_TIE(1)));
                 A32_TS(3);
             } else if constexpr (ND32 == 3) {
                 A32_TRG(1, 0, 1);
-                A32_DKV_STEP(0, (void)0);
+                A32_DKV_STEP(0, A32_FIRST);
                 A32_TRG(0, 0, 2);
                 A32_DKV_STEP(1, A32_WAIT(4, A32_TIE(1)));
                 A32_TRG(1, 1, 0);
@@ -558,22 +600,28 @@
                 elementwise(IC<2>{});
                 elementwise(IC<3>{});
                 A32_TRG(0, 1, 1);
-                A32_DKV_STEP(3, (void)0);
+                A32_NEXT_RC;
+                A32_DKV_STEP(3, A32_FIRST_PF);
                 A32_TRG(1, 1, 2);
-                A32_DKV_STEP(4, A32_WAIT(4, A32_TIE(0)));
+                A32_DKV_STEP(4, A32_WAITN(4 + PF, A32_TIE(0)));
                 A32_DKV_STEP(5, A32_WAIT(0, A32_TIE(1)));
             } else {
                 A32_TRG(1, 0, 1);
-                A32_DKV_STEP(0, (void)0);
+                A32_DKV_STEP(0, A32_FIRST);
                 A32_TRG(0, 1, 0);
                 A32_DKV_STEP(1, A32_WAIT(4, A32_TIE(1)));
                 elementwise(IC<2>{});
                 elementwise(IC<3>{});
                 A32_TRG(1, 1, 1);
-                A32_DKV_STEP(2, (void)0);
+                A32_NEXT_RC;
+                A32_DKV_STEP(2, A32_FIRST_PF);
                 A32_DKV_STEP(3, A32_WAIT(0, A32_TIE(1)));
             }
 #undef A32_DKV_STEP
+#undef A32_NEXT_RC
+#undef A32_FIRST_PF
+#undef A32_FIRST
+#undef A32_WAITN
 #undef A32_TIE
 #undef A32_TRG
         });
@@ -590,6 +638,7 @@
         }
         cur ^= 1;
     }
+#undef A32_RC_READ
     store_rows<DH>(dk + (int64_t)b * S * lddk + (int64_t)h * DH, lddk, ki, S, dkacc, EXPL ? 1.f : 0.5f * scale, hi);
     store_rows<DH>(dv + (int64_t)b * S * lddv + (int64_t)h * DH, lddv, ki, S, dvacc, 1.f, hi);
 #ifdef A32_TIMELINE
@@ -1173,11 +1222,18 @@
 int lrp_attn32_dq(const AttnCall& c) {
     using namespace attn32;
     const bool expl = c.eps_mask != 0.f || c.eps_qk != 0.f;
+    if (c.rc != nullptr) {
+        A32_FOR_DH(c.d, {
+            launch_dq<dq_kernel<false, DH, true>>(c, NWQ, 2 * (2 * (size_t)TILE), (const bf16_t*)c.ofw, c.ldo, c.Dout, c.cos_t, c.sin_t, c.rc);
+        })
+        return lrp_check_launch();
+    }
     if (c.d == 256)
         lrp_with_bool(expl, [&](auto ex) { launch_dq<d256::dq256_kernel<decltype(ex)::value>>(c, d256::NW2, 2 * (2 * (size_t)d256::TILE2)); });
     else A32_FOR_DH(c.d, {
         lrp_with_bool(expl, [&](auto ex) {
-            launch_dq<dq_kernel<decltype(ex)::value, DH>>(c, NWQ, 2 * (2 * (size_t)TILE), (const bf16_t*)c.ofw, c.ldo, c.Dout, c.cos_t, c.sin_t);
+            launch_dq<dq_kernel<decltype(ex)::value, DH>>(c, NWQ, 2 * (2 * (size_t)TILE), (const bf16_t*)c.ofw, c.ldo, c.Dout, c.cos_t, c.sin_t,
+                                                          (float*)nullptr);
         });
     })
     return lrp_check_launch();
@@ -1189,6 +1245,13 @@
     const size_t lds = (wide ? 2 * (2 * (size_t)d256::TILE2 + 512) + (size_t)d256::NW2 * 32 * d256::KP2 : 2 * (2 * (size_t)TILE + 512) + (size_t)NW * 32 * KP) +
                        (iv ? (size_t)((c.S + 31) / 32) * 16 : 0);
     if (lds > A32_LDS_MAX) return LRP_ESHAPE;
+    if (c.rc != nullptr) {
+        AttnCall r = c;
+        r.lse = c.rc;
+        r.D = c.rc + (int64_t)c.B * c.Hq * c.S;
+        A32_FOR_DH(c.d, { lrp_with_bool(iv, [&](auto ivf) { launch_dkv<dkv_kernel<false, DH, decltype(ivf)::value, true>>(r, NW, lds); }); })
+        return lrp_check_launch();
+    }
     if (wide) lrp_with_bool(expl, [&](auto ex) { launch_dkv<d256::dkv256_kernel<decltype(ex)::value>>(c, d256::NW2, lds); });
     else A32_FOR_DH(c.d, {
         lrp_with_bool(expl, [&](auto ex) {
diff --git a/lrp-explains-transformers_amd/csrc/attention32_tiles.hpp b/lrp-explains-transformers_amd/csrc/attention32_tiles.hpp
--- a/lrp-explains-transformers_amd/csrc/attention32_tiles.hpp
+++ b/lrp-explains-transformers_amd/csrc/attention32_tiles.hpp
@@ -83,6 +83,11 @@
 #pragma unroll
     for (int i = 0; i < 16; ++i) z[i] = 0.f;
     return z;
+}
+LRP_DEVICE f32x16 join16(const f32x4 (&a)[4]) {
+    typedef __attribute__((ext_vector_type(8))) float f32x8;
+    const f32x8 lo = __builtin_shufflevector(a[0], a[1], 0, 1, 2, 3, 4, 5, 6, 7), hi = __builtin_shufflevector(a[2], a[3], 0, 1, 2, 3, 4, 5, 6, 7);
+    return __builtin_shufflevector(lo, hi, 0, 1, 2, 3, 4, 5, 6, 7, 8, 9, 10, 11, 12, 13, 14, 15);
 }
 LRP_DEVICE bf16x8 pack8(const f32x16& x, int j) {
     bf16x8 r;
diff --git a/lrp-explains-transformers_amd/csrc/common.hpp b/lrp-explains-transformers_amd/csrc/common.hpp
--- a/lrp-explains-transformers_amd/csrc/common.hpp
+++ b/lrp-explains-transformers_amd/csrc/common.hpp
@@ -251,6 +251,7 @@
     void* o;  float* lse_out;  int64_t ldo;  const void* v_t;
     void* dq;  int64_t lddq;  const void* k_t;
     const void* ofw;  float* Dout;  const float *cos_t, *sin_t;
+    float* rc;
     void *dk, *dv;  int64_t lddk, lddv;  const void *q_t, *gho_t;
 };
 
diff --git a/lrp-explains-transformers_amd/engine.py b/lrp-explains-transformers_amd/engine.py
--- a/lrp-explains-transformers_amd/engine.py
+++ b/lrp-explains-transformers_amd/engine.py
@@ -209,6 +209,7 @@
     Gho = ops.gemm_nn_rs(Gs1, W["wo"], alloc("half", 1, M, 0, torch.float32)[0], new("Gho", nq * d))
     q, k, v = st["qkr"][:, : nq * d], st["qkr"][:, nq * d:], st["qkv"][:, nqk:]
     D = alloc("D", B * nq, S, 0, torch.float32).view(B, nq, S)
+    rc = alloc("rc", 2 * B * nq, S, 0, torch.float32).view(2, B, nq, S) if ops.attn_rc_ok(dt, d) else None
     Aqkv, dk_h, dv_h = new("Aqkv", nqkv, pt["Aqkv"]), new("dk_h", nq * d), new("dv_h", nq * d)
     if heads is not None:
         heads("out", st["o"], Gho, scale=2.0)
@@ -217,8 +218,8 @@
     if attn_map is not None:
         attn_map(q, k, v, Gho, st["lse"], 2.0, row_iv)
     if qk_norm is not None:
-        dq = ops.attn_bwd_dq_d(q, k, v, Gho, st["o"], st["lse"], D, new("dq", nq * d), B, S, nq, nk, d, scale, row_iv=row_iv)
-        ops.attn_bwd_dkv(q, k, v, None, Gho, None, st["lse"], D, dk_h, dv_h, B, S, nq, nk, d, scale, 0.0, 0.0, row_iv=row_iv)
+        dq = ops.attn_bwd_dq_d(q, k, v, Gho, st["o"], st["lse"], D, new("dq", nq * d), B, S, nq, nk, d, scale, row_iv=row_iv, rc=rc)
+        ops.attn_bwd_dkv(q, k, v, None, Gho, None, st["lse"], D, dk_h, dv_h, B, S, nq, nk, d, scale, 0.0, 0.0, row_iv=row_iv, rc=rc)
         if heads is not None:
             heads("q", q, dq)
             heads("k", k, dk_h, nq // nk)
@@ -227,8 +228,8 @@
         if weights is not None:
             weights("qkv", Aqkv, st["h"], W["wqkv"], rs=st["rstd1"])
         return ops.gemm_nn_rs_res(Aqkv, W["wqkv"], st["rstd1"], Gs1, new("Gh", H))
-    ops.attn_bwd_dq_d(q, k, v, Gho, st["o"], st["lse"], D, Aqkv[:, : nq * d], B, S, nq, nk, d, scale, row_iv=row_iv, rope=(cos, sin))
-    ops.attn_bwd_dkv(q, k, v, None, Gho, None, st["lse"], D, dk_h, dv_h, B, S, nq, nk, d, scale, 0.0, 0.0, row_iv=row_iv)
+    ops.attn_bwd_dq_d(q, k, v, Gho, st["o"], st["lse"], D, Aqkv[:, : nq * d], B, S, nq, nk, d, scale, row_iv=row_iv, rope=(cos, sin), rc=rc)
+    ops.attn_bwd_dkv(q, k, v, None, Gho, None, st["lse"], D, dk_h, dv_h, B, S, nq, nk, d, scale, 0.0, 0.0, row_iv=row_iv, rc=rc)
     if heads is not None:
         heads("q", q, Aqkv[:, : nq * d], rope=(cos, sin))
         heads("k", k, dk_h, nq // nk)
@@ -240,7 +241,7 @@
     return ops.gemm_nn_rs_res(Aqkv, W["wqkv"], st["rstd1"], Gs1, new("Gh", H))
 
 
-FUSED_SCRATCH = frozenset(("ssq", "m", "half", "Agu", "Gs1", "Gho", "D", "Aqkv", "dk_h", "dv_h", "dq"))
+FUSED_SCRATCH = frozenset(("ssq", "m", "half", "Agu", "Gs1", "Gho", "D", "rc", "Aqkv", "dk_h", "dv_h", "dq"))
 
 
 
diff --git a/lrp-explains-transformers_amd/ops.py b/lrp-explains-transformers_amd/ops.py
--- a/lrp-explains-transformers_amd/ops.py
+++ b/lrp-explains-transformers_amd/ops.py
@@ -1268,11 +1268,24 @@
     return bool(PREP_FUSION and dtype in _DT and lib.lrp_attn_bwd_dq_d_ok(_DT[dtype], d))
 
 
-def attn_bwd_dq_d(q, k, v, Gho, o, lse, D, dq, B, S, Hq, Hkv, d, scale, causal=True, window=0, row_iv=None, rope=None):
+ATTN_RC = True
+
+
+def attn_rc_ok(dtype, d):
+    return bool(ATTN_RC and dtype == torch.bfloat16 and d in (64, 96, 128))
+
+
+def attn_bwd_dq_d(q, k, v, Gho, o, lse, D, dq, B, S, Hq, Hkv, d, scale, causal=True, window=0, row_iv=None, rope=None, rc=None):
     same(q, k, v, Gho, o, dq)
-    f32(lse, D)
+    f32(lse, D, rc)
     cs, sn = rope if rope is not None else (None, None)
     f32(cs, sn)
+    if rc is not None:
+        assert rc.is_contiguous() and rc.numel() == 2 * B * Hq * S, "rc is [2, B, Hq, S]"
+        check(lib.lrp_attn_bwd_dq_d_rc(p(q), p(k), p(v), p(Gho), p(o), p(lse), p(D), p(dq), B, S, Hq, Hkv, d, q.stride(0), k.stride(0), v.stride(0),
+                                       Gho.stride(0), o.stride(0), dq.stride(0), scale, int(causal), window, *_iv(row_iv, B, S), p(cs), p(sn), dt(q),
+                                       stream(), p(rc)), "lrp_attn_bwd_dq_d_rc")
+        return dq
     check(lib.lrp_attn_bwd_dq_d(p(q), p(k), p(v), p(Gho), p(o), p(lse), p(D), p(dq), B, S, Hq, Hkv, d, q.stride(0), k.stride(0), v.stride(0),
                                 Gho.stride(0), o.stride(0), dq.stride(0), scale, int(causal), window, *_iv(row_iv, B, S), p(cs), p(sn), dt(q),
                                 stream()), "lrp_attn_bwd_dq_d")
@@ -1290,9 +1303,16 @@
 
 
 def attn_bwd_dkv(q, k, v, q_t, Gho, Gho_t, lse, D, dk_h, dv_h, B, S, Hq, Hkv, d, scale, eps_mask, eps_qk, causal=True,
-                 window=0, q_begin=0, row_iv=None):
+                 window=0, q_begin=0, row_iv=None, rc=None):
     same(q, k, v, q_t, Gho, Gho_t, dk_h, dv_h)
-    f32(lse, D)
+    f32(lse, D, rc)
+    if rc is not None:
+        assert rc.is_contiguous() and rc.numel() == 2 * B * Hq * S, "rc is [2, B, Hq, S]"
+        check(lib.lrp_attn_bwd_dkv_rc(p(q), p(k), p(v), p(q_t), p(Gho), p(Gho_t), p(lse), p(D), p(dk_h), p(dv_h), B, S, Hq, Hkv, d,
+                                      q.stride(0), k.stride(0), v.stride(0), q_t.stride(2) if q_t is not None else 0, Gho.stride(0),
+                                      dk_h.stride(0), dv_h.stride(0), scale, eps_mask, eps_qk, int(causal), window, q_begin, *_iv(row_iv, B, S),
+                                      dt(q), stream(), p(rc)), "lrp_attn_bwd_dkv_rc")
+        return dk_h, dv_h
     check(lib.lrp_attn_bwd_dkv(p(q), p(k), p(v), p(q_t), p(Gho), p(Gho_t), p(lse), p(D), p(dk_h), p(dv_h), B, S, Hq, Hkv, d,
                                q.stride(0), k.stride(0), v.stride(0), q_t.stride(2) if q_t is not None else 0, Gho.stride(0),
                                dk_h.stride(0),
```
